# NIFTy-PPL/NIFTy

Hardware: AMD Instinct MI355X
Metric: MGVI iters/sec on 1024^3 RGSpace CorrelatedField, 8 samples; achieved HBM GB/s (higher is better)
Workload: dtype f32

## Files before the change

include/niftyk.h:

```cpp
#ifndef NIFTYK_H
#define NIFTYK_H
#include <stddef.h>
#include <stdint.h>

#ifdef __cplusplus
extern "C" {
#endif

typedef enum {
  NK_OK = 0,
  NK_ERR_INVALID = -1,
  NK_ERR_UNSUPPORTED = -2,
  NK_ERR_RUNTIME = -3,
  NK_ERR_NOMEM = -4
} nk_status;

typedef enum { NK_F32 = 0, NK_F64 = 1 } nk_dtype;

#define NK_HARTLEY_NON_CANONICAL 0
#define NK_HARTLEY_CANONICAL 1

enum { NK_PRO_PLAIN = 0, NK_PRO_AMP = 1, NK_PRO_AMP_JVP = 2, NK_PRO_MUL = 3 };
enum { NK_EPI_AFFINE = 0, NK_EPI_MUL = 1, NK_EPI_VJP = 2, NK_EPI_LIKELIHOOD = 3, NK_EPI_NONLIN = 4 };
enum { NK_LH_GAUSS = 0, NK_LH_POISSON = 1 };
enum { NK_NL_ID = 0, NK_NL_EXP = 1, NK_NL_SIGMOID = 2 };

typedef struct nk_fuse {
  int pro;
  const void* in;
  const void* in2;
  const int32_t* pidx;
  const double* amp;
  const double* damp;
  int epi;
  void* out;
  double scale;
  double offset;
  const void* mul;
  double mul_scalar;
  const void* xi;
  const void* addend;
  double addend_scale;
  int accumulate;
  double* abar;
  int lh_kind, nonlin;
  const void* data;
  const void* icov;
  double icov_scalar;
  void* out2;
  double* value;
  const void* afield;
  const void* dampT;
  int abar_copies;
  int64_t abar_stride;
  const void* dafield;
  double* w8;
  int field_octant;
  int value_slots;
  const int32_t* pidx_octant;
  const void* cg_r;
  const double* cg_scal;
  double* w8max;
  int pipe_chunks;
  void* const* pipe_wait;
  void* const* pipe_record;
  double* wfull;
  int io32;
  const void* carry1;
  const void* carry2;
} nk_fuse;

typedef struct nk_plan nk_plan;

const char* nk_last_error(void);
int nk_version(void);

int nk_plan_create(nk_plan** plan, int ndim, const int64_t* shape, int dtype, int64_t batch);
int nk_plan_destroy(nk_plan* plan);
size_t nk_plan_workspace_bytes(const nk_plan* plan);
int nk_hartley(const nk_plan* plan, const void* in, void* out, double scale, int convention, void* workspace,
               void* stream);
int nk_hartley_fused(const nk_plan* plan, const nk_fuse* fuse, int convention, void* workspace, void* stream);
int nk_plan_pipe_ok(const nk_plan* plan, int chunks);
int nk_plan_sandwich(const nk_plan* plan);
int nk_hartley_sandwich(const nk_plan* plan, const nk_fuse* fuse, double scale_first, int convention, void* workspace,
                        void* stream);
int nk_hartley_sandwich_pair(const nk_plan* plan, const nk_fuse* fuse_a, const nk_fuse* fuse_b, double scale_first,
                             int convention, void* workspace_a, void* workspace_b, void* stream);
int nk_fftn(const nk_plan* plan, const void* in, void* out, int inverse, double scale, void* workspace,
            void* stream);

int nk_profile_enable(int on);
int nk_profile_collect(double* ms, int64_t* count);

int nk_vdot(int64_t n, const void* a, const void* b, int dtype, double* result, int accumulate, void* stream);

int64_t nk_red_unit(int64_t n, int dtype);
int nk_red_layout(int64_t unit_elems, int k_local, int k_global, int seg_units, int seg_stride, int seg_off,
                  double* units_out);
int nk_red_finish(const double* units, int k_global, int nred, double* result, int accumulate, void* stream);
int nk_sum(int64_t n, const void* a, int dtype, double* result, int accumulate, void* stream);
int nk_stats(int64_t n, const void* a, int dtype, double* result3, void* stream);

enum { NK_OP_ADD = 0, NK_OP_SUB = 1, NK_OP_MUL = 2, NK_OP_DIV = 3 };
int nk_binary(int op, int64_t n, const void* a, double ascalar, const void* b, double bscalar, void* out,
              int dtype, void* stream);
int nk_cplx_muldiv(int64_t n, const void* a, int akind, double asr, double asi, const void* b, int bkind, double bsr,
                   double bsi, int conj_b, int divide, void* out, int dtype, void* stream);
int nk_cplx_pointwise(int fn, int64_t n, const void* x, void* out, int dtype, void* stream);
int nk_axpby(int64_t n, double alpha, const void* x, double beta, const void* y, void* out, int dtype,
             void* stream);
int nk_axpby_sqnorm(int64_t n, double alpha, const void* x, double beta, const void* y, void* out, int dtype, double* result,
                    int accumulate, void* stream);
int nk_pointwise(int fn, double param, int64_t n, const void* x, void* fx, void* dfx, int dtype, void* stream);
int nk_clip(double lo, double hi, int64_t n, const void* x, void* fx, void* dfx, int dtype, void* stream);
int nk_gather(int64_t n, const void* table, const int32_t* pidx, void* out, int dtype, void* stream);
int nk_scatter_add(int64_t n, const void* in, const int32_t* pidx, int64_t nbins, void* bins, int dtype,
                   void* stream);

int nk_csr_rowsum(int64_t nrows, const int64_t* rowptr, const int32_t* col, const float* wgt, const void* x, void* y,
                  int dtype, int lanes, void* stream);
int nk_spmv(int64_t nrows, const int64_t* rowptr, const int32_t* col, const float* wgt, const void* x, void* y, int dtype,
            void* stream);
int nk_spmv_t(int64_t nrows, const int64_t* rowptr, const int32_t* col, const float* wgt, const void* y, double* x64,
              int dtype, void* stream);

typedef struct nk_tiled_csr {
  int64_t n_rows, n_slots;
  int32_t n_items, ny, nx, th, tw;
  const int32_t* item_tile;
  const int64_t* item_blk;
  const int32_t* blk_slot;
  const int64_t* row_slot;
  const uint16_t* loc;
  const float* wgt;
} nk_tiled_csr;
int nk_tiled_rowsum(const nk_tiled_csr* m, int count, const void* const* x, void* const* y, double* scratch, int dtype,
                    void* stream);

int nk_roll(int ndim, const int64_t* shape, const int64_t* shift, int elem_bytes, const void* in, void* out, void* stream);

int nk_bluestein_rows(int64_t rows, int n, int m, const void* in, const void* w, const void* bhat_br, const void* tw, void* out,
                      double scale, int in_real, int out_hartley, int dtype, void* stream);

int nk_cumsum(int64_t n, const void* in, void* out, int reverse, int dtype, void* stream);

int nk_cplx_rows(int64_t rows, int64_t in_cols, int64_t out_cols, const void* a, const void* w, void* out, int mode,
                 double scale, int sgn, int dtype, void* stream);

int nk_fold_copies(int64_t n, int copies, int64_t stride, const double* src, double* dst, void* stream);

int nk_octant_expand(int ndim, const int64_t* shape, const void* table, const int32_t* pidx, void* field, int dtype,
                     int compact, void* stream);
int nk_octant_scatter(int ndim, const int64_t* shape, const double* w8, const int32_t* pidx, double* abar,
                      int merge_swapped_lines, void* stream);
int nk_octant_expand_k2(int ndim, const int64_t* shape, const double* table, const int32_t* bin_k2, int64_t nb, void* dense,
                        void* field8, int dtype, const int32_t* line_order, void* stream);
int nk_octant_scatter_k2(int ndim, const int64_t* shape, const double* w8, const int32_t* pidx, const int32_t* bin_k2,
                         int64_t nb, double* scratch, double* abar, const double* w8max, void* stream);
int nk_segment_sum(int64_t nseg, const int32_t* rowptr, const int32_t* perm, const double* src, double* dst, int accumulate,
                   void* stream);
int nk_plan_octant_vjp(const nk_plan* plan);

int nk_pindex_from_k2(int ndim, const int64_t* shape, const int32_t* k2table, int32_t* pidx, int64_t* rho,
                      void* stream);

int nk_cg_curv(int64_t n, const void* d, const void* q, int dtype, double* scal, int accumulate, void* stream);
int nk_cg_update(int64_t n, void* x, void* r, const void* d, const void* q, const void* b, int dtype,
                 double* scal, int accumulate, void* stream);
int nk_cg_update_dr(int64_t n, void* x, void* r, const void* d, const void* q, int dtype, double* scal, int accumulate,
                    void* stream);
int nk_cg_direction(int64_t n, void* d, const void* r, int dtype, double* scal, int roll, void* stream);

typedef struct nk_product {
  int nsub;
  int64_t size[3];
  const int32_t* pidx[3];
  const double* tab[3];
  const double* dtab[3];
  const double* scale;
  const double* dscale;
} nk_product;
int nk_product_field(const nk_product* p, int tangent, void* out, int dtype, void* stream);
int nk_mirror_combine(int ndim, const int64_t* shape, const int* group, int nsub, const double* coef, const void* in,
                      void* out, double scale, double offset, int dtype, void* stream);
size_t nk_product_marginal_scratch(const nk_product* p, int which);
int nk_product_marginal(const nk_product* p, int which, const double* w, double* scratch, double* marg, void* stream);

int nk_amp_forward(int nb, const double* geo, const double* hyp, const double* lat, double* state, double* amp,
                   void* stream);
int nk_amp_jvp(int nb, const double* geo, const double* hyp, const double* lat, double* state, const double* dlat,
               double* damp, void* stream);
int nk_amp_vjp(int nb, const double* geo, const double* hyp, const double* lat, double* state, const double* abar,
               double* latbar, void* stream);

int64_t nk_pcg64_normal_scratch_bytes(int64_t n, int attempt);
int nk_pcg64_normal(const uint64_t* state, const uint64_t* inc, int64_t n, double mean, double std, void* out, int dtype,
                    void* scratch, int64_t scratch_bytes, int attempt, uint64_t* status, void* stream);
int64_t nk_pcg64_fixed_scratch_bytes(void);
int nk_pcg64_uniform(const uint64_t* state, const uint64_t* inc, int64_t n, double low, double high, void* out, int dtype,
                     void* scratch, void* stream);
int nk_pcg64_pm1(const uint64_t* state, const uint64_t* inc, int64_t n, void* out, int dtype, int complex_units, void* scratch,
                 void* stream);

int64_t nk_pcg64_integers_scratch_bytes(int64_t nthreads);
int nk_pcg64_integers(const uint64_t* state, const uint64_t* inc, int64_t n, int64_t low, uint64_t rng, int64_t nthreads, int64_t* out,
                      void* scratch, uint64_t* status, void* stream);

#define NK_MAX_BATCH 8
int nk_plan_batch_ok(const nk_plan* plan);
int nk_hartley_fused_batch(const nk_plan* plan, const nk_fuse* fuse, int count, int convention, void* const* workspace,
                           void* stream);
int nk_amp_forward_batch(int nb, const double* geo, const double* hyp, int count, const double* const* lat,
                         double* const* state, double* const* amp, void* stream);
int nk_amp_jvp_batch(int nb, const double* geo, const double* hyp, int count, const double* const* lat, double* const* state,
                     const double* const* dlat, double* const* damp, void* stream);
int nk_amp_vjp_batch(int nb, const double* geo, const double* hyp, int count, const double* const* lat, double* const* state,
                     const double* const* abar, double* const* latbar, void* stream);
int nk_gather_batch(int64_t n, int count, const void* const* table, const int32_t* pidx, void* const* out, int dtype,
                    void* stream);
int nk_csr_rowsum_batch(int64_t nrows, const int64_t* rowptr, const int32_t* col, const float* wgt, int count,
                        const void* const* x, void* const* y, int dtype, int lanes, void* stream);
int nk_axpby_batch(int64_t n, int count, const double* alpha, const void* const* x, const double* beta,
                   const void* const* y, void* const* out, int dtype, void* stream);
int nk_axpby_sqnorm_batch(int64_t n, int count, const double* alpha, const void* const* x, const double* beta,
                          const void* const* y, void* const* out, int dtype, double* const* result, int accumulate,
                          void* stream);
int nk_binary_batch(int op, int64_t n, int count, const void* const* a, const double* ascalar, const void* const* b,
                    const double* bscalar, void* const* out, int dtype, void* stream);
int nk_vdot_batch(int64_t n, int count, const void* const* a, const void* const* b, int dtype, double* const* result,
                  int accumulate, void* stream);
int nk_sum_tree(int64_t n, int count, const void* const* term, void* out, int dtype, void* stream);
int nk_cg_curv_batch(int64_t n, int count, const void* const* d, const void* const* q, int dtype, double* const* scal,
                     int accumulate, void* stream);
int nk_cg_update_batch(int64_t n, int count, void* const* x, void* const* r, const void* const* d, const void* const* q,
                       const void* const* b, int dtype, double* const* scal, int accumulate, void* stream);
int nk_cg_update_dr_batch(int64_t n, int count, void* const* x, void* const* r, const void* const* d,
                          const void* const* q, int dtype, double* const* scal, int accumulate, void* stream);
int nk_cg_direction_batch(int64_t n, int count, void* const* d, const void* const* r, int dtype, double* const* scal,
                          int roll, void* stream);

// ... 25 lines not shown
```

nifty_amd/_lib.py:

```python
import ctypes
import os

_HERE = os.path.dirname(os.path.abspath(__file__))
LIB_PATH = os.environ.get("NK_LIB_PATH") or os.path.join(_HERE, "csrc", "libniftyk.so")

NK_OK, NK_ERR_INVALID, NK_ERR_UNSUPPORTED, NK_ERR_RUNTIME, NK_ERR_NOMEM = 0, -1, -2, -3, -4
NK_F32, NK_F64 = 0, 1
PRO_PLAIN, PRO_AMP, PRO_AMP_JVP, PRO_MUL = 0, 1, 2, 3
EPI_AFFINE, EPI_MUL, EPI_VJP, EPI_LIKELIHOOD, EPI_NONLIN = 0, 1, 2, 3, 4
LH_GAUSS, LH_POISSON = 0, 1
NL_ID, NL_EXP, NL_SIGMOID = 0, 1, 2
OP_ADD, OP_SUB, OP_MUL, OP_DIV = 0, 1, 2, 3

_vp, _i, _i64, _d, _sz = ctypes.c_void_p, ctypes.c_int, ctypes.c_int64, ctypes.c_double, ctypes.c_size_t


class Fuse(ctypes.Structure):

    _fields_ = [
        ("pro", _i), ("in_", _vp), ("in2", _vp), ("pidx", _vp), ("amp", _vp), ("damp", _vp),
        ("epi", _i), ("out", _vp), ("scale", _d), ("offset", _d), ("mul", _vp), ("mul_scalar", _d),
        ("xi", _vp), ("addend", _vp), ("addend_scale", _d), ("accumulate", _i), ("abar", _vp), ("lh_kind", _i), ("nonlin", _i), ("data", _vp),
        ("icov", _vp), ("icov_scalar", _d), ("out2", _vp), ("value", _vp),
        ("afield", _vp), ("dampT", _vp), ("abar_copies", _i), ("abar_stride", _i64), ("dafield", _vp), ("w8", _vp),
        ("field_octant", _i), ("value_slots", _i), ("pidx_octant", _vp), ("cg_r", _vp), ("cg_scal", _vp), ("w8max", _vp),
        ("pipe_chunks", _i), ("pipe_wait", _vp), ("pipe_record", _vp), ("wfull", _vp), ("io32", _i), ("carry1", _vp), ("carry2", _vp),
    ]


class Product(ctypes.Structure):

    _fields_ = [("nsub", _i), ("size", _i64 * 3), ("pidx", _vp * 3), ("tab", _vp * 3), ("dtab", _vp * 3), ("scale", _vp),
                ("dscale", _vp)]


class TiledCsr(ctypes.Structure):

    _fields_ = [("n_rows", _i64), ("n_slots", _i64), ("n_items", ctypes.c_int32), ("ny", ctypes.c_int32), ("nx", ctypes.c_int32),
                ("th", ctypes.c_int32), ("tw", ctypes.c_int32), ("item_tile", _vp), ("item_blk", _vp), ("blk_slot", _vp),
                ("row_slot", _vp), ("loc", _vp), ("wgt", _vp)]


class NufftPlan(ctypes.Structure):

    _i32 = ctypes.c_int32
    _fields_ = [("ndim", _i32), ("w", _i32), ("beta", _d), ("n", _i32 * 3), ("nmodes", _i32 * 3), ("tile", _i32 * 3),
                ("ntiles", _i32 * 3), ("reach", _i32 * 3), ("m", _i64), ("u", _vp), ("perm", _vp), ("bin_start", _vp),
                ("n_items", _i64), ("item", _vp), ("n_split", _i64), ("split_tile", _vp), ("split_slab", _vp), ("corr", _vp)]


SIGNATURES = {
    "nk_last_error": (ctypes.c_char_p, []),
    "nk_version": (_i, []),
    "nk_plan_create": (_i, [ctypes.POINTER(_vp), _i, ctypes.POINTER(_i64), _i, _i64]),
    "nk_plan_destroy": (_i, [_vp]),
    "nk_plan_workspace_bytes": (_sz, [_vp]),
    "nk_hartley": (_i, [_vp, _vp, _vp, _d, _i, _vp, _vp]),
    "nk_hartley_fused": (_i, [_vp, ctypes.POINTER(Fuse), _i, _vp, _vp]),
    "nk_plan_sandwich": (_i, [_vp]),
    "nk_plan_pipe_ok": (_i, [_vp, _i]),
    "nk_hartley_sandwich": (_i, [_vp, ctypes.POINTER(Fuse), _d, _i, _vp, _vp]),
    "nk_hartley_sandwich_pair": (_i, [_vp, ctypes.POINTER(Fuse), ctypes.POINTER(Fuse), _d, _i, _vp, _vp, _vp]),
    "nk_fftn": (_i, [_vp, _vp, _vp, _i, _d, _vp, _vp]),
    "nk_profile_enable": (_i, [_i]),
    "nk_profile_collect": (_i, [_vp, _vp]),
    "nk_vdot": (_i, [_i64, _vp, _vp, _i, _vp, _i, _vp]),
    "nk_product_field": (_i, [ctypes.POINTER(Product), _i, _vp, _i, _vp]),
    "nk_mirror_combine": (_i, [_i, ctypes.POINTER(_i64), ctypes.POINTER(_i), _i, ctypes.POINTER(_d), _vp, _vp, _d, _d, _i, _vp]),
    "nk_product_marginal_scratch": (_sz, [ctypes.POINTER(Product), _i]),
    "nk_product_marginal": (_i, [ctypes.POINTER(Product), _i, _vp, _vp, _vp, _vp]),
    "nk_red_unit": (_i64, [_i64, _i]),
    "nk_red_layout": (_i, [_i64, _i, _i, _i, _i, _i, _vp]),
    "nk_red_finish": (_i, [_vp, _i, _i, _vp, _i, _vp]),
    "nk_sum": (_i, [_i64, _vp, _i, _vp, _i, _vp]),
    "nk_stats": (_i, [_i64, _vp, _i, _vp, _vp]),
    "nk_binary": (_i, [_i, _i64, _vp, _d, _vp, _d, _vp, _i, _vp]),
    "nk_cplx_muldiv": (_i, [_i64, _vp, _i, _d, _d, _vp, _i, _d, _d, _i, _i, _vp, _i, _vp]),
    "nk_cplx_pointwise": (_i, [_i, _i64, _vp, _vp, _i, _vp]),
    "nk_axpby": (_i, [_i64, _d, _vp, _d, _vp, _vp, _i, _vp]),
    "nk_axpby_sqnorm": (_i, [_i64, _d, _vp, _d, _vp, _vp, _i, _vp, _i, _vp]),
    "nk_pointwise": (_i, [_i, _d, _i64, _vp, _vp, _vp, _i, _vp]),
    "nk_clip": (_i, [_d, _d, _i64, _vp, _vp, _vp, _i, _vp]),
    "nk_gather": (_i, [_i64, _vp, _vp, _vp, _i, _vp]),
    "nk_scatter_add": (_i, [_i64, _vp, _vp, _i64, _vp, _i, _vp]),
    "nk_octant_expand": (_i, [_i, ctypes.POINTER(_i64), _vp, _vp, _vp, _i, _i, _vp]),
    "nk_octant_scatter": (_i, [_i, ctypes.POINTER(_i64), _vp, _vp, _vp, _i, _vp]),
    "nk_octant_expand_k2": (_i, [_i, ctypes.POINTER(_i64), _vp, _vp, _i64, _vp, _vp, _i, _vp, _vp]),
    "nk_segment_sum": (_i, [_i64, _vp, _vp, _vp, _vp, _i, _vp]),
    "nk_octant_scatter_k2": (_i, [_i, ctypes.POINTER(_i64), _vp, _vp, _vp, _i64, _vp, _vp, _vp, _vp]),
    "nk_plan_octant_vjp": (_i, [_vp]),
    "nk_fold_copies": (_i, [_i64, _i, _i64, _vp, _vp, _vp]),
    "nk_cumsum": (_i, [_i64, _vp, _vp, _i, _i, _vp]),
    "nk_cplx_rows": (_i, [_i64, _i64, _i64, _vp, _vp, _vp, _i, _d, _i, _i, _vp]),
    "nk_csr_rowsum": (_i, [_i64, _vp, _vp, _vp, _vp, _vp, _i, _i, _vp]),
    "nk_tiled_rowsum": (_i, [ctypes.POINTER(TiledCsr), _i, _vp, _vp, _vp, _i, _vp]),
    "nk_bluestein_rows": (_i, [_i64, _i, _i, _vp, _vp, _vp, _vp, _vp, _d, _i, _i, _i, _vp]),
    "nk_roll": (_i, [_i, ctypes.POINTER(_i64), ctypes.POINTER(_i64), _i, _vp, _vp, _vp]),
    "nk_spmv": (_i, [_i64, _vp, _vp, _vp, _vp, _vp, _i, _vp]),
    "nk_spmv_t": (_i, [_i64, _vp, _vp, _vp, _vp, _vp, _i, _vp]),
    "nk_pindex_from_k2": (_i, [_i, ctypes.POINTER(_i64), _vp, _vp, _vp, _vp]),
    "nk_cg_curv": (_i, [_i64, _vp, _vp, _i, _vp, _i, _vp]),
    "nk_cg_update": (_i, [_i64, _vp, _vp, _vp, _vp, _vp, _i, _vp, _i, _vp]),
    "nk_cg_update_dr": (_i, [_i64, _vp, _vp, _vp, _vp, _i, _vp, _i, _vp]),
    "nk_pcg64_normal_scratch_bytes": (_i64, [_i64, _i]),
    "nk_pcg64_normal": (_i, [_vp, _vp, _i64, _d, _d, _vp, _i, _vp, _i64, _i, _vp, _vp]),
    "nk_pcg64_fixed_scratch_bytes": (_i64, []),
    "nk_pcg64_uniform": (_i, [_vp, _vp, _i64, _d, _d, _vp, _i, _vp, _vp]),
    "nk_pcg64_pm1": (_i, [_vp, _vp, _i64, _vp, _i, _i, _vp, _vp]),
    "nk_pcg64_integers_scratch_bytes": (_i64, [_i64]),
    "nk_pcg64_integers": (_i, [_vp, _vp, _i64, _i64, ctypes.c_uint64, _i64, _vp, _vp, _vp, _vp]),
    "nk_cg_direction": (_i, [_i64, _vp, _vp, _i, _vp, _i, _vp]),
    "nk_amp_forward": (_i, [_i, _vp, _vp, _vp, _vp, _vp, _vp]),
    "nk_amp_jvp": (_i, [_i, _vp, _vp, _vp, _vp, _vp, _vp, _vp]),
    "nk_amp_vjp": (_i, [_i, _vp, _vp, _vp, _vp, _vp, _vp, _vp]),
    "nk_nufft_spread": (_i, [ctypes.POINTER(NufftPlan), _vp, _vp, _vp, _i, _vp]),
    "nk_nufft_interp": (_i, [ctypes.POINTER(NufftPlan), _vp, _vp, _i, _vp]),
    "nk_nufft_crop": (_i, [ctypes.POINTER(NufftPlan), _vp, _vp, _i, _vp]),
    "nk_nufft_pad": (_i, [ctypes.POINTER(NufftPlan), _vp, _i, _vp, _i, _vp]),
    "nk_plan_batch_ok": (_i, [_vp]),
    "nk_hartley_fused_batch": (_i, [_vp, ctypes.POINTER(Fuse), _i, _i, _vp, _vp]),
    "nk_amp_forward_batch": (_i, [_i, _vp, _vp, _i, _vp, _vp, _vp, _vp]),
    "nk_amp_jvp_batch": (_i, [_i, _vp, _vp, _i, _vp, _vp, _vp, _vp, _vp]),
    "nk_amp_vjp_batch": (_i, [_i, _vp, _vp, _i, _vp, _vp, _vp, _vp, _vp]),
    "nk_gather_batch": (_i, [_i64, _i, _vp, _vp, _vp, _i, _vp]),
    "nk_csr_rowsum_batch": (_i, [_i64, _vp, _vp, _vp, _i, _vp, _vp, _i, _i, _vp]),
    "nk_axpby_batch": (_i, [_i64, _i, _vp, _vp, _vp, _vp, _vp, _i, _vp]),
    "nk_axpby_sqnorm_batch": (_i, [_i64, _i, _vp, _vp, _vp, _vp, _vp, _i, _vp, _i, _vp]),
    "nk_binary_batch": (_i, [_i, _i64, _i, _vp, _vp, _vp, _vp, _vp, _i, _vp]),
    "nk_vdot_batch": (_i, [_i64, _i, _vp, _vp, _i, _vp, _i, _vp]),
    "nk_sum_tree": (_i, [_i64, _i, _vp, _vp, _i, _vp]),
    "nk_cg_curv_batch": (_i, [_i64, _i, _vp, _vp, _i, _vp, _i, _vp]),
    "nk_cg_update_batch": (_i, [_i64, _i, _vp, _vp, _vp, _vp, _vp, _i, _vp, _i, _vp]),
    "nk_cg_update_dr_batch": (_i, [_i64, _i, _vp, _vp, _vp, _vp, _i, _vp, _i, _vp]),
    "nk_cg_direction_batch": (_i, [_i64, _i, _vp, _vp, _i, _vp, _i, _vp]),
}
MAX_BATCH = 8


def ptr_array(tensors):
    return (_vp * len(tensors))(*[None if t is None else t.data_ptr() for t in tensors])


def double_array(values):
    return (_d * len(values))(*[float(v) for v in values])

_lib = None


class NiftykError(RuntimeError):
    pass


def load():
    global _lib
    if _lib is not None:
        return _lib
    if not os.path.exists(LIB_PATH):
        raise NiftykError(
            f"{LIB_PATH} not found: the HIP extension is not built. Run `python -c 'import __graft_entry__ as g; "
            "g.build()'` (hipcc --offload-arch=gfx950). nifty_amd has no CPU fallback for device fields."
        )
    lib = ctypes.CDLL(LIB_PATH)
    for name, (res, args) in SIGNATURES.items():
        fn = getattr(lib, name)
        fn.restype = res
        fn.argtypes = args
    _lib = lib
    return lib


def check(rc, what=""):
    if rc == NK_OK:
        return
    msg = load().nk_last_error().decode(errors="replace")
    text = f"{what}: {msg}" if what else msg
    if rc == NK_ERR_INVALID:
        raise ValueError(text)
    if rc == NK_ERR_UNSUPPORTED:
        raise NotImplementedError(text)
    if rc == NK_ERR_NOMEM:
        raise MemoryError(text)
    raise NiftykError(text)
```

nifty_amd/backend.py:

```python
import ctypes
import math
import os

import numpy as np
import torch

from . import _lib as L
from . import config

_DT = {torch.float32: L.NK_F32, torch.float64: L.NK_F64}
_plans = {}


_raw_stream = getattr(torch._C, "_cuda_getCurrentRawStream", None)


_current_device = torch.cuda.current_device


def _stream():
    if _raw_stream is not None:
        return _raw_stream(_current_device())
    return torch.cuda.current_stream().cuda_stream

# ... 82 lines not shown
    except NotImplementedError:
        _unsupported.add(key)
        return False
    return True


_chirps = {}
_CHIRP_MAX = 1 << 14


def _chirp(n, cdt, inverse, device):
    key = (n, cdt, bool(inverse), device.index)
    ent = _chirps.get(key)
    if ent is None:
        m = 1 << (2 * n - 2).bit_length()
        if m > _CHIRP_MAX:
            raise NotImplementedError(f"axis of length {n} is too long for the chirp-z fallback")
        k = torch.arange(n, dtype=torch.int64)
        ang = (k * k % (2 * n)).to(torch.float64) * (math.pi / n)
        w = torch.polar(torch.ones(n, dtype=torch.float64), ang if inverse else -ang)
        b = torch.zeros(m, dtype=torch.complex128)
        b[:n] = w.conj()
        b[m - n + 1:] = w.conj()[1:].flip(0)
        w, b = w.to(cdt).to(device), b.to(cdt).to(device)
        rdt = torch.float32 if cdt == torch.complex64 else torch.float64
        get_plan((m,), rdt, 1, device)
        ent = _chirps[key] = (m, w, fftn(b, ndim=1))
    return ent


BLUESTEIN_LDS_BYTES = 64 * 1024
_blu_tables = {}


def _bluestein_tables(n, m, cdt, inverse, device):
    key = (n, m, cdt, bool(inverse), device.index)
    ent = _blu_tables.get(key)
    if ent is None:
        k = np.arange(n, dtype=np.int64)
        ang = (k * k % (2 * n)).astype(np.float64) * (np.pi / n)
        w = np.exp(1j * ang if inverse else -1j * ang)
        b = np.zeros(m, dtype=np.complex128)
        b[:n] = w.conj()
        b[m - n + 1:] = w.conj()[1:][::-1]
        bhat = np.fft.fft(b)
        bits = m.bit_length() - 1
        rev = np.zeros(m, dtype=np.int64)
        for bit in range(bits):
            rev |= ((np.arange(m) >> bit) & 1) << (bits - 1 - bit)
        tw = np.exp(-2j * np.pi * np.arange(m // 2) / m)
        npdt = np.complex64 if cdt == torch.complex64 else np.complex128
        ent = _blu_tables[key] = tuple(torch.from_numpy(np.ascontiguousarray(a.astype(npdt))).to(device) for a in (w, bhat[rev], tw))
    return ent


def cplx_rows(a, w, in_cols, out_cols, mode, scale=1.0, sgn=1):
    _require_device(a, w)
    rows = a.numel() // max(1, in_cols)
    if mode == 2:
        rdt = torch.float32 if a.dtype == torch.complex64 else torch.float64
        out = torch.empty(a.shape[:-1] + (out_cols,), dtype=rdt, device=a.device)
    else:
        cdt = a.dtype if a.is_complex() else (torch.complex64 if a.dtype == torch.float32 else torch.complex128)
        out = torch.empty(a.shape[:-1] + (out_cols,), dtype=cdt, device=a.device)
    code = 0 if out.dtype in (torch.float32, torch.complex64) else 1
    L.check(L.load().nk_cplx_rows(rows, in_cols, out_cols, a.data_ptr(), ptr(w), out.data_ptr(), mode, float(scale),
                                  int(sgn), code, _stream()), "nk_cplx_rows")
    return out


def _fft_last_axis_any(z, inverse, real_in=False, hartley=0, scale=1.0):
    n = z.shape[-1]
    rdt = z.dtype if real_in else (torch.float32 if z.dtype == torch.complex64 else torch.float64)
    cdt = torch.complex64 if rdt == torch.float32 else torch.complex128
    batch = z.numel() // max(1, n)
    m = 1 << max(2, (2 * n - 2).bit_length())
    native = n == 1 or z.numel() == 0 or plan_supported((n,), rdt, batch, z.device)
    if (not native and m * (8 if rdt == torch.float32 else 16) <= BLUESTEIN_LDS_BYTES and os.environ.get("NK_BLUESTEIN", "1") != "0"):
        w, bhat_br, tw = _bluestein_tables(n, m, cdt, inverse, z.device)
        out = torch.empty(z.shape, dtype=rdt if hartley else cdt, device=z.device)
        L.check(L.load().nk_bluestein_rows(batch, n, m, z.data_ptr(), w.data_ptr(), bhat_br.data_ptr(), tw.data_ptr(), out.data_ptr(),
                                           float(scale) if hartley else 1.0, 1 if real_in else 0, int(hartley),
                                           0 if rdt == torch.float32 else 1, _stream()), "nk_bluestein_rows")
        return out
    if real_in:
        z = cplx_rows(z, None, n, n, 1)
    if n == 1 or z.numel() == 0:
        res = z.clone()
    elif native:
        res = fftn(z, ndim=1, inverse=inverse)
    else:
        if m > _CHIRP_MAX or not plan_supported((m,), rdt, batch, z.device) or not plan_supported((m,), rdt, 1, z.device):
            raise NotImplementedError(f"axis of length {n} is too long for the chirp-z fallback")
        m, w, fb = _chirp(n, z.dtype, inverse, z.device)
        a = cplx_rows(z, w, n, m, 0)
        p = cplx_rows(fftn(a, ndim=1), fb, m, m, 0)
        c = fftn(p, ndim=1, inverse=True, scale=1.0 / m)
        res = cplx_rows(c, w, m, n, 0)
    return cplx_rows(res, None, n, n, 2, scale, hartley) if hartley else res


def _fft_any(z, ndim, inverse, real_in=False, hartley=0, scale=1.0):
    first, last = z.dim() - ndim, z.dim() - 1
    for ax in range(first, z.dim()):
        z = _fft_last_axis_any(z.movedim(ax, -1).contiguous(), inverse, real_in=real_in and ax == first,
                               hartley=hartley if ax == last else 0, scale=scale).movedim(-1, ax)
    return z.contiguous()


def _convention():
    return 0 if config.get("hartley_convention") == "non_canonical_hartley" else 1


def hartley(x, ndim=None, scale=1.0, out=None):
    _require_device(x)
    x = x.contiguous()
    ndim = x.dim() if ndim is None else ndim
    shape = x.shape[x.dim() - ndim:]
    batch = x.numel() // max(1, int(torch.Size(shape).numel()))
    if not plan_supported(shape, x.dtype, batch, x.device):
        h = _fft_any(x, ndim, False, real_in=True, hartley=1 if _convention() == 0 else -1, scale=scale)
        return h if out is None else out.copy_(h)
    plan = get_plan(shape, x.dtype, batch, x.device)
    out = torch.empty_like(x) if out is None else out
    L.check(L.load().nk_hartley(plan.handle, x.data_ptr(), out.data_ptr(), float(scale), _convention(),
                                plan.workspace.data_ptr(), _stream()), "nk_hartley")
    return out


def hartley_fused(plan, fuse):
    if plan.device.index != _current_device():
        _wrong_device(plan.device.index)
    L.check(L.load().nk_hartley_fused(plan.handle, ctypes.byref(fuse), _convention(), plan.workspace.data_ptr(),
                                      _stream()), "nk_hartley_fused")


def plan_sandwich(plan):
    return bool(L.load().nk_plan_sandwich(plan.handle))


def hartley_sandwich(plan, fuse, scale_first):
    if plan.device.index != _current_device():
        _wrong_device(plan.device.index)
    L.check(L.load().nk_hartley_sandwich(plan.handle, ctypes.byref(fuse), float(scale_first), _convention(),
                                         plan.workspace.data_ptr(), _stream()), "nk_hartley_sandwich")


def hartley_sandwich_pair(plan, fuse_a, fuse_b, scale_first, workspace_b):
    if plan.device.index != _current_device():
        _wrong_device(plan.device.index)
    L.check(L.load().nk_hartley_sandwich_pair(plan.handle, ctypes.byref(fuse_a), ctypes.byref(fuse_b), float(scale_first),
                                              _convention(), plan.workspace.data_ptr(), workspace_b.data_ptr(), _stream()),
            "nk_hartley_sandwich_pair")


def fftn(x, ndim=None, inverse=False, scale=1.0):
    _require_device(x)
    if not x.is_complex():
        raise TypeError("fftn expects a complex tensor")
    x = x.contiguous()
    ndim = x.dim() if ndim is None else ndim
    shape = x.shape[x.dim() - ndim:]
    batch = x.numel() // max(1, int(torch.Size(shape).numel()))
    rdt = torch.float32 if x.dtype == torch.complex64 else torch.float64
    if not plan_supported(shape, rdt, batch, x.device):
        f = _fft_any(x, ndim, inverse)
        return f if float(scale) == 1.0 else cplx_rows(f, None, f.shape[-1], f.shape[-1], 0, scale)
    plan = get_plan(shape, rdt, batch, x.device)
    out = torch.empty_like(x)
    L.check(L.load().nk_fftn(plan.handle, torch.view_as_real(x).data_ptr(), torch.view_as_real(out).data_ptr(),
                             1 if inverse else 0, float(scale), plan.workspace.data_ptr(), _stream()), "nk_fftn")
    return out


def new_scalar(device, n=1):
    return torch.zeros(n, dtype=torch.float64, device=device)


def vdot(a, b, result=None, accumulate=False):
    _require_device(a, b)
    if a.numel() != b.numel() or a.dtype != b.dtype:
        raise ValueError("vdot: shape/dtype mismatch")
    result = new_scalar(a.device) if result is None else result
    L.check(L.load().nk_vdot(a.numel(), a.data_ptr(), b.data_ptr(), dtype_code(a), result.data_ptr(),
                             1 if accumulate else 0, _stream()), "nk_vdot")
    return result


def vsum(a, result=None, accumulate=False):
    _require_device(a)
    result = new_scalar(a.device) if result is None else result
    L.check(L.load().nk_sum(a.numel(), a.data_ptr(), dtype_code(a), result.data_ptr(), 1 if accumulate else 0,
                            _stream()), "nk_sum")
    return result


def binary(op, a, b, out=None):
    ta, tb = torch.is_tensor(a), torch.is_tensor(b)
    ref = a if ta else b
    _require_device(ref)
    if ta and tb and (a.shape != b.shape or a.dtype != b.dtype):
        raise ValueError("binary: shape/dtype mismatch")
    out = torch.empty_like(ref) if out is None else out
    L.check(L.load().nk_binary(op, ref.numel(), ptr(a) if ta else 0, 0.0 if ta else float(a), ptr(b) if tb else 0,
                               0.0 if tb else float(b), out.data_ptr(), dtype_code(ref), _stream()), "nk_binary")
    return out


def _cplx_operand(x, cdt):
    if torch.is_tensor(x):
        if x.is_complex():
            return x.to(cdt).contiguous(), 0, 0.0, 0.0
        rdt = torch.float32 if cdt == torch.complex64 else torch.float64
        return x.to(rdt).contiguous(), 1, 0.0, 0.0
    z = complex(x)
    return None, 2, z.real, z.imag


def cplx_muldiv(a, b, divide=False, conj_b=False):
    tensors = [t for t in (a, b) if torch.is_tensor(t)]
    _require_device(*tensors)
    wide = any(t.dtype in (torch.complex128, torch.float64) for t in tensors)
    cdt = torch.complex128 if wide else torch.complex64
    ta, ka, ar, ai = _cplx_operand(a, cdt)
    tb, kb, br, bi = _cplx_operand(b, cdt)
    shape = tensors[0].shape
    if any(t.shape != shape for t in tensors):
        raise ValueError("cplx_muldiv: shape mismatch")
    out = torch.empty(shape, dtype=cdt, device=tensors[0].device)
    L.check(L.load().nk_cplx_muldiv(out.numel(), ptr(ta), ka, ar, ai, ptr(tb), kb, br, bi, int(bool(conj_b)), int(bool(divide)),
                                    out.data_ptr(), 0 if cdt == torch.complex64 else 1, _stream()), "nk_cplx_muldiv")
    return out


CPLX_POINTWISE = {"exp": 0, "log": 1, "sqrt": 2, "reciprocal": 3, "conjugate": 4, "abs": 5, "absolute": 5}


def cplx_pointwise(op, x):
    _require_device(x)
    x = x.contiguous()
    fn = CPLX_POINTWISE[op]
    rdt = torch.float32 if x.dtype == torch.complex64 else torch.float64
    out = torch.empty(x.shape, dtype=rdt if fn == 5 else x.dtype, device=x.device)
    L.check(L.load().nk_cplx_pointwise(fn, x.numel(), x.data_ptr(), out.data_ptr(), 0 if x.dtype == torch.complex64 else 1,
                                       _stream()), "nk_cplx_pointwise")
    return out


def axpby(alpha, x, beta=0.0, y=None, out=None):
    _require_device(x, y)
    out = torch.empty_like(x) if out is None else out
    L.check(L.load().nk_axpby(x.numel(), float(alpha), x.data_ptr(), float(beta), ptr(y), out.data_ptr(), dtype_code(x),
                              _stream()), "nk_axpby")
    return out


def axpby_sqnorm(alpha, x, beta, y, result, accumulate=False):
    _require_device(x, y, result)
    out = torch.empty_like(x)
    L.check(L.load().nk_axpby_sqnorm(x.numel(), float(alpha), x.data_ptr(), float(beta), y.data_ptr(), out.data_ptr(),
                                     dtype_code(x), result.data_ptr(), 1 if accumulate else 0, _stream()), "nk_axpby_sqnorm")
    return out


POINTWISE = {"exp": 0, "log": 1, "sqrt": 2, "tanh": 3, "sigmoid": 4, "reciprocal": 5, "power": 6, "abs": 7,
             "absolute": 7, "log1p": 8, "expm1": 9, "arctan": 10, "sin": 11, "cos": 12, "tan": 13, "sinc": 14, "log10": 15,
             "sinh": 16, "cosh": 17, "sign": 18, "softplus": 19, "exponentiate": 20, "unitstep": 21, "clip": 22}


def pointwise(name, x, param=0.0, want_derivative=False, param2=None):
    _require_device(x)
    fx = torch.empty_like(x)
    dfx = torch.empty_like(x) if want_derivative else None
    if name == "clip":
        lo = -math.inf if param is None else float(param)
        hi = math.inf if param2 is None else float(param2)
        L.check(L.load().nk_clip(lo, hi, x.numel(), x.data_ptr(), fx.data_ptr(), ptr(dfx), dtype_code(x), _stream()), "nk_clip")
    else:
        L.check(L.load().nk_pointwise(POINTWISE[name], float(param), x.numel(), x.data_ptr(), fx.data_ptr(), ptr(dfx),
                                      dtype_code(x), _stream()), "nk_pointwise")
    return (fx, dfx) if want_derivative else fx


def gather(table, pidx, out_shape, out=None):
    _require_device(table, pidx)
    out = torch.empty(out_shape, dtype=table.dtype, device=table.device) if out is None else out
    L.check(L.load().nk_gather(out.numel(), table.data_ptr(), pidx.data_ptr(), out.data_ptr(), dtype_code(table),
                               _stream()), "nk_gather")
    return out


def scatter_add(x, pidx, nbins):
    _require_device(x, pidx)
    bins = torch.zeros(nbins, dtype=torch.float64, device=x.device)
    L.check(L.load().nk_scatter_add(x.numel(), x.data_ptr(), pidx.data_ptr(), nbins, bins.data_ptr(), dtype_code(x),
                                    _stream()), "nk_scatter_add")
    return bins


def lanes_for(nnz, nrows):
    avg = nnz / max(1, nrows)
    return 1 if avg <= 4 else 4 if avg <= 32 else 16 if avg <= 256 else 64


BIN_PLAN_MAX = 1 << 28

# ... 217 lines not shown
    lib = L.load()
    status = torch.empty(2, dtype=torch.int64, device=device)

    def draw(state, inc, need, lo, span, nthreads):
        words = (ctypes.c_uint64 * 4)(state >> 64, state & (2**64 - 1), inc >> 64, inc & (2**64 - 1))
        scratch = torch.empty(lib.nk_pcg64_integers_scratch_bytes(nthreads), dtype=torch.uint8, device=device)
        dst = out[n - need:]
        L.check(lib.nk_pcg64_integers(ctypes.addressof(words), ctypes.addressof(words) + 16, need, lo, span, nthreads, dst.data_ptr(),
                                      scratch.data_ptr(), status.data_ptr(), _stream()), "nk_pcg64_integers")
        used, err = status.cpu().tolist()
        return dst, int(used), bool(err & 2)

    first, _ = _bounded_integers(rng, low, high, n, draw)
    if n and int(high) == int(low):
        out.fill_(int(low))
    elif first:
        out[:len(first)] = torch.tensor(first, dtype=torch.int64)
    return out.reshape(tuple(shape))


def pcg64_normal(rng, mean, std, shape, dtype, device):
    import ctypes

    import numpy as np

    bg = rng.bit_generator
    st = bg.state
    if st.get("bit_generator") != "PCG64":
        raise TypeError("pcg64_normal needs a numpy Generator over PCG64 (np.random.default_rng)")
    if float(std) < 0:
        raise ValueError("scale < 0")
    n = int(np.prod(shape, dtype=np.int64)) if len(tuple(shape)) else 1
    out = torch.empty(tuple(shape), dtype=dtype, device=device)
    _require_device(out)
    if n == 0:
        return out
    state, inc = int(st["state"]["state"]), int(st["state"]["inc"])
    words = (ctypes.c_uint64 * 4)(state >> 64, state & (2**64 - 1), inc >> 64, inc & (2**64 - 1))
    status = torch.empty(2, dtype=torch.int64, device=device)
    lib = L.load()
    for attempt in range(9):
        nbytes = lib.nk_pcg64_normal_scratch_bytes(n, attempt)
        scratch = torch.empty(nbytes, dtype=torch.uint8, device=device)
        L.check(lib.nk_pcg64_normal(ctypes.addressof(words), ctypes.addressof(words) + 16, n, float(mean), float(std),
                                    out.data_ptr(), dtype_code(out), scratch.data_ptr(), nbytes, attempt,
                                    status.data_ptr(), _stream()), "nk_pcg64_normal")
        consumed, err = status.cpu().tolist()
        del scratch
        if err == 0:
            break
        if err & 1:
            raise RuntimeError("nk_pcg64_normal: chain merge failed")
    else:
        raise RuntimeError("nk_pcg64_normal: scratch sizing failed")
    st["state"]["state"] = _pcg64_advanced(state, inc, int(consumed))
    bg.state = st
    return out


def _pcg64_words(rng):
    bg = rng.bit_generator
    st = bg.state
    if st.get("bit_generator") != "PCG64":
        raise TypeError("needs a numpy Generator over PCG64 (np.random.default_rng)")
    import ctypes

    state, inc = int(st["state"]["state"]), int(st["state"]["inc"])
    words = (ctypes.c_uint64 * 4)(state >> 64, state & (2**64 - 1), inc >> 64, inc & (2**64 - 1))
    return bg, st, state, inc, words


def pcg64_uniform(rng, low, high, shape, dtype, device):
    import ctypes

    import numpy as np

    bg, st, state, inc, words = _pcg64_words(rng)
    n = int(np.prod(shape, dtype=np.int64)) if len(tuple(shape)) else 1
    out = torch.empty(tuple(shape), dtype=dtype, device=device)
    _require_device(out)
    if n == 0:
        return out
    lib = L.load()
    scratch = torch.empty(lib.nk_pcg64_fixed_scratch_bytes(), dtype=torch.uint8, device=device)
    L.check(lib.nk_pcg64_uniform(ctypes.addressof(words), ctypes.addressof(words) + 16, n, float(low), float(high),
                                 out.data_ptr(), dtype_code(out), scratch.data_ptr(), _stream()), "nk_pcg64_uniform")
    st["state"]["state"] = _pcg64_advanced(state, inc, n)
    bg.state = st
    return out


def pcg64_pm1(rng, shape, dtype, device, complex_units=False):
    import ctypes

    import numpy as np

    n = int(np.prod(shape, dtype=np.int64)) if len(tuple(shape)) else 1
    cdt = {torch.float32: torch.complex64, torch.float64: torch.complex128}[dtype]
    out = torch.empty(tuple(shape), dtype=cdt if complex_units else dtype, device=device)
    _require_device(out)
    if n == 0:
        return out
    flat = (torch.view_as_real(out) if complex_units else out).reshape(-1)
    width = 2 if complex_units else 1
    done = 0
    if rng.bit_generator.state["has_uint32"]:
        v = int(rng.integers(0, 4 if complex_units else 2))
        first = ([1, 0], [0, 1], [-1, 0], [0, -1])[v] if complex_units else [2 * v - 1]
        flat[:width] = torch.tensor(first, dtype=dtype, device=device)
        done = 1
    m = n - done
    if m > 0:
        bg, st, state, inc, words = _pcg64_words(rng)
        lib = L.load()
        scratch = torch.empty(lib.nk_pcg64_fixed_scratch_bytes(), dtype=torch.uint8, device=device)
        L.check(lib.nk_pcg64_pm1(ctypes.addressof(words), ctypes.addressof(words) + 16, m, flat[done * width:].data_ptr(),
                                 _DT[dtype], 1 if complex_units else 0, scratch.data_ptr(), _stream()), "nk_pcg64_pm1")
        nraw = (m + 1) // 2
        if m % 2:
            st["state"]["state"] = _pcg64_advanced(state, inc, nraw - 1)
            bg.state = st
            last = int(bg.random_raw(1)[0])
            st = bg.state
            st["has_uint32"], st["uinteger"] = 1, last >> 32
            bg.state = st
        else:
            st["state"]["state"] = _pcg64_advanced(state, inc, nraw)
            st["has_uint32"], st["uinteger"] = 0, 0
            bg.state = st
    return out


def _runs_on_operand_device(fn):
    import functools

    @functools.wraps(fn)
    def wrapper(*args, **kw):
        for a in args:
            if torch.is_tensor(a):
                if a.is_cuda and a.device.index != _current_device():
                    with torch.cuda.device(a.device):
                        return fn(*args, **kw)
                break
            if isinstance(a, (Plan, PlanView)):
                if a.device.index != _current_device():
                    with torch.cuda.device(a.device):
                        return fn(*args, **kw)
                break
        return fn(*args, **kw)

    return wrapper


for _name in ("cplx_rows", "cplx_pointwise", "hartley", "hartley_fused", "hartley_sandwich", "hartley_sandwich_pair", "fftn", "vdot", "vsum", "binary", "axpby",
              "axpby_sqnorm",
              "pointwise", "gather", "scatter_add", "bin_plan", "bin_sum", "spmv", "spmv_t", "stats", "cumsum"):
    globals()[_name] = _runs_on_operand_device(globals()[_name])
del _name
```

nifty_amd/csrc/nk_fft.hip:

```cpp
#include <hip/hip_runtime.h>

#include <algorithm>

#include <cstdio>
#include <cstring>
#include <new>

#include "nk_fft_batch.h"

#include <mutex>
#include <vector>
using ProfScope = NkProfScope;
thread_local const NkBatchCtx* t_batch = nullptr;

template <typename T>
__device__ __forceinline__ void nk_run_stages(C2<T>* lds, int tid, int nthr, const NkLinePlan& lp, const NkTile& tl,
                                              const C2<T>* __restrict__ tw) {
  int L = lp.n;
  for (int s = 0; s < lp.nstage; ++s) {
    const int R = lp.radix[s];
    NK_STAGE_DISPATCH(R, lds, tid, nthr, lp, tl, L, tw, s)
    L /= R;
    __syncthreads();
  }
// ... 125 lines not shown
  NkFuse fs = f;
  pf.blk0 = 0;
  if (pf.a_cnt > 0) {
    if (pf.g.batch != 1 || (xmap_env & 4)) return nk_set_error(NK_ERR_UNSUPPORTED, "staged final pass: batch 1, natural block order");
    pf.blk0 = (int64_t)pf.a0 * pf.tiles_per_a;
    blocks = (int64_t)pf.a_cnt * pf.tiles_per_a;
    const int64_t off = pf.blk0 * ((CT::THREADS + 63) / 64);
    if (fs.value_slots > 0) {
      if (fs.value) fs.value += off;
      if (fs.w8max) fs.w8max += off;
      fs.value_slots = fs.value_slots > off ? (int)(fs.value_slots - off) : 0;
      if (fs.value_slots == 0) return nk_set_error(NK_ERR_RUNTIME, "final pass: more wavefronts than reduction slots (nk_value_slot_count)");
    }
  }
  if (fs.value_slots > 0 && blocks * ((CT::THREADS + 63) / 64) > fs.value_slots)
    return nk_set_error(NK_ERR_RUNTIME, "final pass: more wavefronts than reduction slots (nk_value_slot_count)");
  if (t_batch != nullptr) {
    if constexpr (nk_twin_final<NL, COUPLES, EC, PAIR>()) {
      if (pf.a_cnt > 0 || pf.g.batch != 1) return nk_set_error(NK_ERR_UNSUPPORTED, "batched final pass: one unstaged grid per member");
      return nk_twin_launch_final<T, NL, COUPLES, EC>(pf, blocks, tw, xmap_env & 4, st);
    } else {
      return nk_set_error(NK_ERR_UNSUPPORTED, "batched final pass: no batched twin of this kernel class");
    }
  }
  return nk_launch<k2_final<T, NL, COUPLES, EC, PAIR>>("k2_final", dim3((unsigned)blocks), dim3(CT::THREADS), CT::LDS_BYTES, st, pf, fs, tw,
                                                       work, xmap_env & 4);
}

template <typename T, int NL>
static int nk_launch_final(const NkPassF& pf, const NkFuse& f, const C2<T>* tw, const C2<T>* work, hipStream_t st) {
  if (nk_knobs().ec_generic && !f.field_octant) {
    if (f.epi == NK_EPI_VJP) return nk_launch_final_c<T, NL, true, -1>(pf, f, tw, work, st);
    return nk_launch_final_c<T, NL, false, -1>(pf, f, tw, work, st);
  }
  if (f.epi == NK_EPI_VJP && f.afield) {
    if constexpr (nk_final_single_2d<T, NL>())
      if (pf.A == 1) return nk_launch_final_c<T, NL, false, 2>(pf, f, tw, work, st);
    return nk_launch_final_c<T, NL, true, 2>(pf, f, tw, work, st);
  }
  if (f.epi == NK_EPI_VJP) return nk_launch_final_c<T, NL, true, -1>(pf, f, tw, work, st);
  if (f.epi == NK_EPI_AFFINE) return nk_launch_final_c<T, NL, false, 0>(pf, f, tw, work, st);
  if (f.epi == NK_EPI_MUL) return nk_launch_final_c<T, NL, false, 1>(pf, f, tw, work, st);
  if (f.epi == NK_EPI_LIKELIHOOD) {
    if constexpr (sizeof(T) == 8)
      if (f.io32) return nk_launch_final_c<T, NL, false, 5>(pf, f, tw, work, st);
    return nk_launch_final_c<T, NL, false, 3>(pf, f, tw, work, st);
  }
  return nk_launch_final_c<T, NL, false, -1>(pf, f, tw, work, st);
}

template <typename T, int NL>
static int nk_launch_final3(const NkPassF& pf, const NkFuse& f, const C2<T>* tw, const C2<T>* work, hipStream_t st) {
  if (f.epi == NK_EPI_VJP && f.afield) return nk_launch_final_c<T, NL, true, 2, 1>(pf, f, tw, work, st);
  if (f.epi == NK_EPI_VJP) return nk_launch_final_c<T, NL, true, -1, 1>(pf, f, tw, work, st);
  if (f.epi == NK_EPI_AFFINE) return nk_launch_final_c<T, NL, false, 0, 1>(pf, f, tw, work, st);
  return nk_launch_final_c<T, NL, false, -1, 1>(pf, f, tw, work, st);
}

template <typename T>
static int nk_dispatch_final3(int nl, const NkPassF& pf, const NkFuse& f, const C2<T>* tw, const C2<T>* work,
                              hipStream_t st) {
  return nk_dispatch_fast(nl, "no fast final pass for this length", [&](auto N) { return nk_launch_final3<T, N()>(pf, f, tw, work, st); });
}

template <typename T>
static int nk_dispatch_final_pair(int nl, const NkPassF& pf, const NkFuse& fa, const NkFuse& fb, const C2<T>* tw,
                                  const C2<T>* worka, const C2<T>* workb, hipStream_t st) {
  return nk_dispatch_fast(nl, "no fast final pass for this length",
                          [&](auto N) { return nk_launch_final_pair<T, N()>(pf, fa, fb, tw, worka, workb, st); });
}

template <typename T>
static int nk_dispatch_final(int nl, const NkPassF& pf, const NkFuse& f, const C2<T>* tw, const C2<T>* work,
                             hipStream_t st) {
  return nk_dispatch_fast(nl, "no fast final pass for this length", [&](auto N) { return nk_launch_final<T, N()>(pf, f, tw, work, st); });
}

template <typename T, int H, bool IS_1D>
static int nk_launch_contig(const NkPassA& pa, const NkFuse& f, const C2<T>* tw, const C2<T>* twr, C2<T>* work,
                            hipStream_t st) {
  using CT = ContigTile<T, H>;
  const int64_t blocks = (pa.nlines + CT::TILE - 1) / CT::TILE;
  return nk_launch<k2_contig<T, H, IS_1D>>("k2_contig", dim3((unsigned)blocks), dim3(CT::THREADS), CT::LDS_BYTES, st, pa, f, tw, twr, work);
}

template <typename T, int N, int MODE, int PC>
static int nk_launch_strided_pc(NkPassS ps, const NkFuse& f, const C2<T>* tw, C2<T>* work, C2<T>* scratch, hipStream_t st) {
  using ST = StridedTile<T, N, nk_strided_cx<MODE, PC>(), MODE>;
  ps.tl.tile = ST::TILE;
  ps.tl.dtile = nk_make_div(ST::TILE);
  ps.tiles_per_slab = (int)(ps.inner / ST::TILE);
  const int64_t blocks = ps.outer * ps.tiles_per_slab;
  const int xmap_env = nk_knobs().xmap;
  const int xmap = MODE == 3 ? (xmap_env & 1) : ((xmap_env & 2) | ((xmap_env & 8) && ps.blo > 0 ? 2 : 0));
  if (t_batch != nullptr) {
    if constexpr (MODE != 3 || !nk_twin_strided<N, PC>()) {
      return nk_set_error(NK_ERR_UNSUPPORTED, "batched strided pass: no batched twin of this kernel class");
    } else {
      return nk_twin_launch_strided<T, N, PC>(ps, blocks, tw, xmap, st);
    }
  }
  return nk_launch<k2_strided<T, N, MODE, PC>>("k2_strided", dim3((unsigned)blocks), dim3(ST::THREADS), ST::LDS_TOTAL, st, ps, f, tw, work,
                                               scratch, xmap);
}

template <typename T, bool IS_1D>
static int nk_dispatch_contig(int h, const NkPassA& pa, const NkFuse& f, const C2<T>* tw, const C2<T>* twr, C2<T>* work,
                              hipStream_t st) {
  return nk_dispatch_fast(h, "no fast contiguous pass for this length",
                          [&](auto N) { return nk_launch_contig<T, N(), IS_1D>(pa, f, tw, twr, work, st); });
}

template <typename T, int N, int MODE>
static int nk_launch_strided(const NkPassS& ps, const NkFuse& f, const C2<T>* tw, C2<T>* work, C2<T>* scratch, hipStream_t st) {
  if constexpr (MODE == 3) {
    if constexpr (sizeof(T) == 8)
      if (f.field_octant && f.pro == NK_PRO_AMP && f.io32) return nk_launch_strided_pc<T, N, MODE, 9>(ps, f, tw, work, scratch, st);
    if (f.field_octant && f.pro == NK_PRO_AMP) return nk_launch_strided_pc<T, N, MODE, 4>(ps, f, tw, work, scratch, st);
    if (f.field_octant && f.pro == NK_PRO_AMP_JVP) return nk_launch_strided_pc<T, N, MODE, 5>(ps, f, tw, work, scratch, st);
    if (f.pro == NK_PRO_PLAIN) return nk_launch_strided_pc<T, N, MODE, 0>(ps, f, tw, work, scratch, st);
    if (f.pro == NK_PRO_MUL) return nk_launch_strided_pc<T, N, MODE, 6>(ps, f, tw, work, scratch, st);
    if (f.pro == NK_PRO_AMP && f.afield) return nk_launch_strided_pc<T, N, MODE, 1>(ps, f, tw, work, scratch, st);
    if (f.pro == NK_PRO_AMP_JVP && f.afield && f.dafield)
      return nk_launch_strided_pc<T, N, MODE, 3>(ps, f, tw, work, scratch, st);
    if (f.pro == NK_PRO_AMP_JVP && f.afield && f.dampT)
      return nk_launch_strided_pc<T, N, MODE, 2>(ps, f, tw, work, scratch, st);
  }
  return nk_launch_strided_pc<T, N, MODE, -1>(ps, f, tw, work, scratch, st);
}

template <typename T, int MODE>
static int nk_dispatch_strided(int n, const NkPassS& ps, const NkFuse& f, const C2<T>* tw, C2<T>* work, C2<T>* scratch,
                               hipStream_t st) {
  return nk_dispatch_fast(n, "no fast strided pass for this length",
                          [&](auto N) { return nk_launch_strided<T, N(), MODE>(ps, f, tw, work, scratch, st); });
}

#ifndef NK_CONTIG3_WAVES
#define NK_CONTIG3_WAVES 0
#endif
#if NK_CONTIG3_WAVES > 0
#define NK_CONTIG3_ATTR __attribute__((amdgpu_waves_per_eu(1, NK_CONTIG3_WAVES)))
#else
#define NK_CONTIG3_ATTR
#endif
template <typename T, int H, int PC>
__global__ void __launch_bounds__((Contig3Tile<T, H>::THREADS)) NK_CONTIG3_ATTR
    k3_contig(NkPass3 p, NkFuse f, const C2<T>* __restrict__ tw, const C2<T>* __restrict__ twr, C2<T>* __restrict__ work) {
  extern __shared__ __align__(16) unsigned char smem[];
  DeviceExec<T, Contig3Tile<T, H>::SC::E> ex;
  nk_contig3_body<T, H, Contig3Tile<T, H>::TILE, PC>(ex, p, f, blockIdx.x, (T*)smem, tw, twr, work);
}

#ifndef NK_QUAD_MAXW_F64_5
#define NK_QUAD_MAXW_F64_5 4
#endif
#ifndef NK_QUAD_MAXW_F64_8
#define NK_QUAD_MAXW_F64_8 8
#endif
#ifndef NK_QUAD_MAXW_F32_5
#define NK_QUAD_MAXW_F32_5 8
#endif
#ifndef NK_QUAD_MAXW_F32_8
#define NK_QUAD_MAXW_F32_8 8
#endif
template <typename T, int PC>
constexpr int nk_quad_max_waves() {
  return sizeof(T) == 8 ? (PC == 8 ? NK_QUAD_MAXW_F64_8 : NK_QUAD_MAXW_F64_5) : (PC == 8 ? NK_QUAD_MAXW_F32_8 : NK_QUAD_MAXW_F32_5);
}
template <typename T, int H, int PC>
__global__ void __launch_bounds__((Contig3Tile<T, H>::QTHREADS))
    k3_contig_quad(NkPass3 p, NkFuse f, const C2<T>* __restrict__ tw, const C2<T>* __restrict__ twr, C2<T>* __restrict__ work) {
  extern __shared__ __align__(16) unsigned char smem[];
  DeviceExec<T, Contig3Tile<T, H>::SC::E> ex;
  nk_contig3_body<T, H, 4, PC, true>(ex, p, f, (int64_t)blockIdx.x + p.blk0, (T*)smem, tw, twr, work, (int)blockIdx.y);
}
template <typename T, int H, int PC, int MAXW>
__global__ void __launch_bounds__((Contig3Tile<T, H>::QTHREADS)) __attribute__((amdgpu_waves_per_eu(1, MAXW)))
    k3_contig_quad_w(NkPass3 p, NkFuse f, const C2<T>* __restrict__ tw, const C2<T>* __restrict__ twr, C2<T>* __restrict__ work) {
  extern __shared__ __align__(16) unsigned char smem[];
  DeviceExec<T, Contig3Tile<T, H>::SC::E> ex;
  nk_contig3_body<T, H, 4, PC, true>(ex, p, f, (int64_t)blockIdx.x + p.blk0, (T*)smem, tw, twr, work, (int)blockIdx.y);
}
template <typename T, int H, int PC>
static constexpr auto nk_quad_kernel() {
  if constexpr (nk_quad_max_waves<T, PC>() < 8)
    return k3_contig_quad_w<T, H, PC, nk_quad_max_waves<T, PC>()>;
  else
    return k3_contig_quad<T, H, PC>;
}

template <typename T, int H, int PC>
static int nk_launch_contig3(const NkPass3& p3, const NkFuse& f, const C2<T>* tw, const C2<T>* twr, C2<T>* work, hipStream_t st) {
  using CT = Contig3Tile<T, H>;
  if constexpr ((PC == 4 || PC == 5 || PC == 7 || PC == 8) && CT::QUAD_OK) {
    if (nk_contig3_quad(p3.nblk, p3.g.ndim)) {
      const int64_t batch = p3.nlines / ((int64_t)p3.g.na * p3.g.nm);
      int64_t qblocks = batch * (p3.g.na / 2 + 1) * (p3.g.nm / 2 + 1);
      if (p3.nblk > 0) {
        if (batch != 1 || p3.blk0 < 0 || p3.blk0 + p3.nblk > qblocks) return nk_set_error(NK_ERR_INVALID, "k3_contig_quad: bad stage range");
        qblocks = p3.nblk;
      }
      const int64_t per = (int64_t)(p3.g.na / 2 + 1) * (p3.g.nm / 2 + 1);
      const int64_t gx = p3.nblk > 0 ? qblocks : per;
      if (gx > 0x7fffffffLL || batch > 65535) return nk_set_error(NK_ERR_UNSUPPORTED, "too many lines for one launch");
      NkPass3 pq = p3;
      pq.dmh = nk_make_div(p3.g.nm / 2 + 1);
      return nk_launch<nk_quad_kernel<T, H, PC>()>("k3_contig_quad", dim3((unsigned)gx, (unsigned)(p3.nblk > 0 ? 1 : batch)), dim3(CT::QTHREADS),
                                                   CT::QLDS_BYTES, st, pq, f, tw, twr, work);
    }
  }
  if (p3.nblk > 0)
    return nk_set_error(NK_ERR_UNSUPPORTED, "nk_fuse.pipe_chunks: the staged first pass exists for the QUAD launches only (3-D plan, "
                                             "octant prologue classes, last axis <= 2048 fp32, NK_CONTIG_QUAD != 0)");
  const int64_t blocks = (p3.nlines + CT::TILE - 1) / CT::TILE;
  if (blocks > 0x7fffffffLL) return nk_set_error(NK_ERR_UNSUPPORTED, "too many lines for one launch");
  return nk_launch<k3_contig<T, H, PC>>("k3_contig", dim3((unsigned)blocks), dim3(CT::THREADS), CT::LDS_BYTES, st, p3, f, tw, twr, work);
}

template <typename T, int H>
static int nk_launch_contig3_pc(const NkPass3& p3, const NkFuse& f, const C2<T>* tw, const C2<T>* twr, C2<T>* work, hipStream_t st) {
  if (f.field_octant && f.pro == NK_PRO_AMP) return nk_launch_contig3<T, H, 4>(p3, f, tw, twr, work, st);
  if (f.field_octant && f.pro == NK_PRO_AMP_JVP && f.cg_r && f.dafield) return nk_launch_contig3<T, H, 8>(p3, f, tw, twr, work, st);
  if (f.field_octant && f.pro == NK_PRO_AMP_JVP && f.pidx_octant && f.dampT) return nk_launch_contig3<T, H, 7>(p3, f, tw, twr, work, st);
  if (f.field_octant && f.pro == NK_PRO_AMP_JVP) return nk_launch_contig3<T, H, 5>(p3, f, tw, twr, work, st);
  if (f.pro == NK_PRO_PLAIN) return nk_launch_contig3<T, H, 0>(p3, f, tw, twr, work, st);
  if (f.pro == NK_PRO_MUL) return nk_launch_contig3<T, H, 6>(p3, f, tw, twr, work, st);
  return nk_launch_contig3<T, H, -1>(p3, f, tw, twr, work, st);
}

template <typename T>
static int nk_dispatch_contig3(int h, const NkPass3& p3, const NkFuse& f, const C2<T>* tw, const C2<T>* twr, C2<T>* work,
                               hipStream_t st) {
  return nk_dispatch_fast(h, "no fast contiguous pass for this length",
                          [&](auto N) { return nk_launch_contig3_pc<T, N()>(p3, f, tw, twr, work, st); });
}

#ifndef NK_MID_CX
#define NK_MID_CX 1
#endif
#ifndef NK_MID_WAVES
#define NK_MID_WAVES 0
#endif
#ifndef NK_MID_PF
#define NK_MID_PF 0
#endif
#ifndef NK_MID_WIDE_XM
#define NK_MID_WIDE_XM 2
#endif
#ifndef NK_MID_WIDE
#define NK_MID_WIDE 0
#endif
#ifndef NK_MID_TWO
#define NK_MID_TWO 1
#endif
#ifndef NK_MID_TWO_MF
#define NK_MID_TWO_MF 0
#endif
template <typename T, int N, bool MF>
struct MidCfg {
  static constexpr bool WIDE = NK_MID_WIDE && SchedW<T, N>::E == 64;
  static constexpr bool TWO = NK_MID_TWO && !WIDE && (!MF || NK_MID_TWO_MF) && sizeof(T) == 4 && Sched<T, N>::E == 32 &&
                              StridedTile<T, N, false, 3>::THREADS == 512 && StridedTile<T, N, false, 3>::LDS_BYTES <= 64 * 1024;
  using ST = StridedTile<T, N, !WIDE && !TWO && NK_MID_CX != 0, WIDE ? 0 : 3>;
  using SC = typename ST::SC;
  static constexpr int XM = WIDE ? NK_MID_WIDE_XM : (ST::CPLX ? 1 : 0);
  static constexpr bool TWC = TWO;
  static constexpr int WAVES = NK_MID_WAVES > 0 ? NK_MID_WAVES : TWO ? 4 : ST::THREADS <= 256 ? 2 : 1;
};
template <typename T, int N, bool MF>
__global__ void __launch_bounds__((MidCfg<T, N, MF>::ST::THREADS), (MidCfg<T, N, MF>::WAVES))
    k3_mid(NkPassM pm, NkFuse f, const C2<T>* __restrict__ tw, C2<T>* __restrict__ work, int64_t nblk, int xmap) {
  extern __shared__ __align__(16) unsigned char smem[];
  using CF = MidCfg<T, N, MF>;
  using ST = typename CF::ST;
  DeviceExecR<MidRegs<T, CF::SC::E, NK_MID_PF != 0>> ex;
  C2<T>* tw_lds = ST::TWLDS ? reinterpret_cast<C2<T>*>(smem + ST::LDS_BYTES) : nullptr;
  nk_mid_body<T, N, ST::TILE, CF::XM, MF, NK_MID_PF != 0, typename CF::SC, CF::TWC>(ex, pm, f, (int64_t)blockIdx.x, (int64_t)gridDim.x,
                                                                                     nblk, xmap, (T*)smem, tw, work, tw_lds);
}

template <typename T, int N, bool MF>
static int nk_launch_mid(NkPassM pm, const NkFuse& f, const C2<T>* tw, C2<T>* work, hipStream_t st) {
  using ST = typename MidCfg<T, N, MF>::ST;
  pm.s.tl.tile = ST::TILE;
  pm.s.tl.dtile = nk_make_div(ST::TILE);
  pm.s.tiles_per_slab = (int)(pm.s.inner / ST::TILE);
  const int64_t blocks = pm.s.outer * pm.s.tiles_per_slab;
  int64_t grid = blocks;
  if (NK_MID_PF) {
    static int cus = 0;
    if (cus == 0) {
      int dev = 0;
      hipDeviceProp_t prop;
      cus = (hipGetDevice(&dev) == hipSuccess && hipGetDeviceProperties(&prop, dev) == hipSuccess) ? prop.multiProcessorCount : 256;
    }
    const int per_cu_env = nk_knobs().mid_wg_per_cu;
    const int per_cu = per_cu_env > 0 ? per_cu_env : (ST::LDS_TOTAL <= 80 * 1024 && ST::THREADS <= 512 ? 2 : 1);
    if (grid > (int64_t)cus * per_cu) grid = (int64_t)cus * per_cu;
  }
  return nk_launch<k3_mid<T, N, MF>>("k3_mid", dim3((unsigned)grid), dim3(ST::THREADS), ST::LDS_TOTAL, st, pm, f, tw, work, blocks,
                                     nk_knobs().xmap & 2);
}

template <typename T>
static int nk_dispatch_mid(int n, const NkPassM& pm, const NkFuse& f, const C2<T>* tw, C2<T>* work, hipStream_t st) {
  return nk_dispatch_fast(n, "no fast strided pass for this length", [&](auto N) {
    return f.mul ? nk_launch_mid<T, N(), true>(pm, f, tw, work, st) : nk_launch_mid<T, N(), false>(pm, f, tw, work, st);
  });
}

struct NkPassCC {
  NkLinePlan lp;
  NkTile tl;
  int64_t nlines;
  int swap;
  double scale;
  NkDiv dn;
};

template <typename T>
__global__ void __launch_bounds__(nk_gen_max_threads<T>()) k_c2c_contig(NkPassCC p, const C2<T>* __restrict__ tw, const C2<T>* __restrict__ in,
// ... 543 lines not shown
  __shared__ double red[4];
  const double* slots = sa.slots[blockIdx.y];
  if (!slots) return;
  double* part = sa.slots[blockIdx.y] + n;
  const int64_t per = (n + gridDim.x - 1) / gridDim.x;
  const int64_t lo = (int64_t)blockIdx.x * per, hi = lo + per < n ? lo + per : n;
  double v = 0.0;
  for (int64_t i = lo + threadIdx.x; i < hi; i += 256) v += slots[i];
  const double s = nk_fold_block_sum(v, red);
  if (threadIdx.x == 0) part[blockIdx.x] = s;
}
__global__ void __launch_bounds__(NK_FOLD_BLOCKS) k_fold_slots_b_b(NkSlotArr sa, int64_t n) {
  __shared__ double red[NK_FOLD_BLOCKS / 64];
  if (!sa.slots[blockIdx.y]) return;
  const double* part = sa.slots[blockIdx.y] + n;
  const double s = nk_fold_block_sum(part[threadIdx.x], red);
  if (threadIdx.x == 0) *sa.value[blockIdx.y] += s;
}

static bool nk_same_class(const nk_fuse& a, const nk_fuse& b) {
  return a.pro == b.pro && a.epi == b.epi && !a.afield == !b.afield && !a.dafield == !b.dafield && !a.dampT == !b.dampT &&
         a.field_octant == b.field_octant && !a.io32 == !b.io32 && !a.w8 == !b.w8 && !a.wfull == !b.wfull &&
         a.abar_copies == b.abar_copies && !a.pidx_octant == !b.pidx_octant;
}

extern "C" int nk_plan_batch_ok(const nk_plan* P) {
  if (!P || !nk_plan_uses_pipeline2(P)) return 0;
  const NkHostPlan& hp = P->hp;
  if (hp.g.ndim != 2 || hp.g.batch != 1) return 0;
  return P->hp.dtype == NK_F32 ? nk_fast_strided_ok<float>(hp.g.na, hp.pc.inner) : nk_fast_strided_ok<double>(hp.g.na, hp.pc.inner);
}

template <typename T>
static int nk_run_hartley_batch(const nk_plan* P, const nk_fuse* fuse, int count, int convention, void* const* workspace,
                                hipStream_t st) {
  const NkHostPlan& hp = P->hp;
  NkBatchCtx bc;
  bc.count = count;
  bc.fuse = fuse;
  for (int m = 0; m < NK_MAX_BATCH; ++m) {
    const int k = m < count ? m : 0;
    bc.wa.work[m] = workspace[k];
    bc.wa.scratch[m] = (char*)workspace[k] + (hp.work_bytes + 255) / 256 * 256;
  }
  NkPipe2 q = nk_pipe2_setup(hp, convention == NK_HARTLEY_CANONICAL ? -1 : 1, nk_knobs().work_blo, nk_knobs().work_pad);
  {
    const int64_t smax = q.s1.ss > q.s0.inner ? q.s1.ss : q.s0.inner;
    if (128 * (smax > q.s1.inner ? smax : q.s1.inner) * (int64_t)sizeof(C2<T>) >= ((int64_t)1 << 32))
      return nk_set_error(NK_ERR_UNSUPPORTED, "transform too large for the 32-bit thread offsets of the strided passes");
  }
  const int64_t n = nk_value_slot_count(hp);
  NkSlotArr sa;
  bool any = false;
  for (int m = 0; m < NK_MAX_BATCH; ++m) {
    sa.slots[m] = nullptr, sa.value[m] = nullptr;
    if (m >= count) {
      bc.final_fuse[m] = fuse[0];
      continue;
    }
    NkFuse f2 = fuse[m];
    if (f2.w8max && f2.w8 && f2.epi == NK_EPI_VJP)
      return nk_set_error(NK_ERR_UNSUPPORTED, "nk_fuse.w8max: only the 3-D final pass reports max |w8|");
    f2.w8max = nullptr;
    if (f2.value && (f2.epi == NK_EPI_LIKELIHOOD || f2.epi == NK_EPI_VJP)) {
      sa.slots[m] = nk_value_slots(hp, workspace[m]);
      sa.value[m] = f2.value;
      f2.value = sa.slots[m];
      f2.value_slots = (int)std::min<int64_t>(n, 0x7fffffff);
      any = true;
    }
    bc.final_fuse[m] = f2;
  }
  struct Scope {
    Scope(const NkBatchCtx* b) { t_batch = b; }
    ~Scope() { t_batch = nullptr; }
  } scope(&bc);
  int rc;
  {
    NkProfScope ps(st, 1, fuse[0].pro, fuse[0].epi, count);
    int n1, n2;
    if (nk_tl_split<T>(hp.g, n1, n2))
      rc = nk_tl_first_axis<T>(q.s1, n1, n2, fuse[0], (const C2<T>*)P->d_tw_t64, (const C2<T>*)(n2 == 64 ? P->d_tw_t64 : P->d_tw_t32),
                               (const C2<T>*)P->d_tw_c, (C2<T>*)bc.wa.work[0], st);
    else
      rc = nk_dispatch_strided<T, 3>(hp.g.na, q.s1, fuse[0], (const C2<T>*)P->d_tw_c, (C2<T>*)bc.wa.work[0], (C2<T>*)bc.wa.scratch[0], st);
  }
  if (rc != NK_OK) return rc;
  if (any) {
    hipLaunchKernelGGL(k_zero_slots_b, dim3(64, count), dim3(256), 0, st, sa, n);
    rc = nk_check_launch("k_zero_slots_b");
    if (rc != NK_OK) return rc;
  }
  {
    NkProfScope ps(st, 3, fuse[0].pro, fuse[0].epi, count);
    rc = nk_dispatch_final<T>(hp.g.nl, q.pf, bc.final_fuse[0], (const C2<T>*)P->d_tw_f, (const C2<T>*)bc.wa.work[0], st);
  }
  if (rc != NK_OK || !any) return rc;
  hipLaunchKernelGGL(k_fold_slots_a_b, dim3(NK_FOLD_BLOCKS, count), dim3(256), 0, st, sa, n);
  hipLaunchKernelGGL(k_fold_slots_b_b, dim3(1, count), dim3(NK_FOLD_BLOCKS), 0, st, sa, n);
  return nk_check_launch("k_fold_slots_b");
}

extern "C" int nk_hartley_fused_batch(const nk_plan* P, const nk_fuse* fuse, int count, int convention, void* const* workspace,
                                      void* stream) {
  if (!P || !fuse || !workspace || count < 1 || count > NK_MAX_BATCH)
    return nk_set_error(NK_ERR_INVALID, "nk_hartley_fused_batch: bad argument (1 <= count <= NK_MAX_BATCH)");
  for (int m = 0; m < count; ++m) {
    const int rc = nk_fused_check(P, fuse + m, convention);
    if (rc != NK_OK) return rc;
    if (!workspace[m]) return nk_set_error(NK_ERR_INVALID, "nk_hartley_fused_batch: every member needs a workspace");
    for (int k = 0; k < m; ++k)
      if (workspace[k] == workspace[m]) return nk_set_error(NK_ERR_INVALID, "nk_hartley_fused_batch: members share a workspace");
    if (!nk_same_class(fuse[0], fuse[m]))
      return nk_set_error(NK_ERR_INVALID, "nk_hartley_fused_batch: the members select different kernel classes");
  }
  hipStream_t st = (hipStream_t)stream;
  if (count == 1 || !nk_plan_batch_ok(P) || !nk_batch_class_ok(P->hp.g, fuse[0])) {
    for (int m = 0; m < count; ++m) {
      const int rc = P->hp.dtype == NK_F32 ? nk_run_hartley<float>(P, fuse[m], convention, workspace[m], st)
                                           : nk_run_hartley<double>(P, fuse[m], convention, workspace[m], st);
      if (rc != NK_OK) return rc;
    }
    return NK_OK;
  }
  if (P->hp.dtype == NK_F32) return nk_run_hartley_batch<float>(P, fuse, count, convention, workspace, st);
  return nk_run_hartley_batch<double>(P, fuse, count, convention, workspace, st);
}

static bool nk_strided_tile_divides(const nk_plan* P, int n, int64_t inner) {
  return P->hp.dtype == NK_F32 ? nk_fast_strided_ok<float>(n, inner) : nk_fast_strided_ok<double>(n, inner);
}
extern "C" int nk_plan_sandwich(const nk_plan* P) {
  if (!P || !nk_plan_uses_pipeline2(P) || !nk_fast_contig_ok(P->hp.g.h)) return 0;
  const NkGeom& g = P->hp.g;
  const int64_t rs = g.h + (P->hp.dtype == NK_F32 ? nk_pipe3_colpad<float>() : nk_pipe3_colpad<double>());
  if (g.ndim == 3 && !nk_strided_tile_divides(P, g.nm, rs)) return 0;
  return nk_strided_tile_divides(P, g.na, g.ndim == 3 ? (int64_t)g.nm * rs : rs) ? 1 : 0;
}

template <typename T>
static bool nk_contig3_quad_ok(int h) {
  return nk_with_fast_size(h, false, [](auto N) { return (bool)Contig3Tile<T, N()>::QUAD_OK; });
}
extern "C" int nk_plan_pipe_ok(const nk_plan* P, int chunks) {
  if (!nk_plan_sandwich(P) || chunks < 2 || (chunks & 1)) return 0;
  const NkGeom& g = P->hp.g;
  if (g.ndim != 3 || g.batch != 1 || g.na % chunks != 0) return 0;
  if (!nk_knobs().contig_quad || (nk_knobs().xmap & 4)) return 0;
  return (P->hp.dtype == NK_F32 ? nk_contig3_quad_ok<float>(g.h) : nk_contig3_quad_ok<double>(g.h)) ? 1 : 0;
}

template <typename T>
static int nk_run_sandwich(const nk_plan* P, const NkFuse& f, double scale_first, int convention, void* workspace, hipStream_t st,
                           bool with_final = true, NkPipe3* q_out = nullptr) {
  const NkHostPlan& hp = P->hp;
  const int sign = convention == NK_HARTLEY_CANONICAL ? -1 : 1;
  const int work_pad = nk_knobs().work_pad;
  const NkPipe3 q = nk_pipe3_setup<T>(hp, sign, work_pad, scale_first * (f.mul_scalar != 0.0 ? f.mul_scalar : 1.0));
  if (q_out) *q_out = q;
  if (nk_pipe3_work_elems(hp.g, nk_pipe3_colpad<T>(), work_pad) * sizeof(C2<T>) > hp.work_bytes)
    return nk_set_error(NK_ERR_RUNTIME, "nk_hartley_sandwich: plan workspace too small");
  if (128 * (q.ss > q.pm.s.inner ? q.ss : q.pm.s.inner) * (int64_t)sizeof(C2<T>) >= ((int64_t)1 << 32))
    return nk_set_error(NK_ERR_UNSUPPORTED, "transform too large for the 32-bit thread offsets of the strided passes");
  C2<T>* work = (C2<T>*)workspace;
  int rc;
  const int C = f.pipe_chunks >= 2 ? f.pipe_chunks : 0;
  if (C) {
    if (hp.g.ndim != 3 || hp.g.batch != 1 || (C & 1) || hp.g.na % C != 0 || !f.field_octant ||
        (f.pro != NK_PRO_AMP && f.pro != NK_PRO_AMP_JVP))
      return nk_set_error(NK_ERR_UNSUPPORTED, "nk_fuse.pipe_chunks: needs a 3-D plan with batch 1, an even chunk count that divides "
                                               "the first axis, and an octant amplitude prologue");
  }
  const int wc = C ? hp.g.na / C : 0;
  if (C) {
    const int Mh = hp.g.nm / 2 + 1;
    for (int j = 0; j < C / 2; ++j) {
      if (f.pipe_wait) {
        hipError_t e = hipStreamWaitEvent(st, (hipEvent_t)f.pipe_wait[j], 0);
        if (e != hipSuccess) return nk_set_hip_error(e, "hipStreamWaitEvent(pipe_wait)");
      }
      NkPass3 p1 = q.p1;
      const int a_lo = j * wc, a_hi = (j == C / 2 - 1) ? hp.g.na / 2 + 1 : (j + 1) * wc;
      p1.blk0 = (int64_t)a_lo * Mh;
      p1.nblk = (int64_t)(a_hi - a_lo) * Mh;
      ProfScope ps(st, 5, f.cg_r ? 4 : f.pro, f.epi);
      rc = nk_dispatch_contig3<T>(hp.g.h, p1, f, (const C2<T>*)P->d_tw_a, (const C2<T>*)P->d_twr_a, work, st);
      if (rc != NK_OK) return rc;
    }
  } else {
    ProfScope ps(st, 5, f.cg_r ? 4 : f.pro, f.epi);
    rc = nk_dispatch_contig3<T>(hp.g.h, q.p1, f, (const C2<T>*)P->d_tw_a, (const C2<T>*)P->d_twr_a, work, st);
    if (rc != NK_OK) return rc;
  }
  if (hp.g.ndim == 3) {
    ProfScope ps(st, 6, f.pro, f.epi);
    rc = nk_dispatch_strided<T, 0>(hp.g.nm, q.s2, f, (const C2<T>*)P->d_tw_b, work, (C2<T>*)nullptr, st);
    if (rc != NK_OK) return rc;
  }
  {
    ProfScope ps(st, 7, f.pro, f.epi);
    rc = nk_dispatch_mid<T>(hp.g.na, q.pm, f, (const C2<T>*)P->d_tw_c, work, st);
  }
  if (rc != NK_OK) return rc;
  if (hp.g.ndim == 3) {
    ProfScope ps(st, 6, f.pro, f.epi);
    rc = nk_dispatch_strided<T, 0>(hp.g.nm, q.s2, f, (const C2<T>*)P->d_tw_b, work, (C2<T>*)nullptr, st);
    if (rc != NK_OK) return rc;
  }
  if (!with_final) return NK_OK;
  ProfScope ps(st, 3, f.pro, f.epi);
  return nk_final_with_slots(hp, workspace, f, st, [&](const NkFuse& f2) {
    if (!C) return nk_dispatch_final3<T>(hp.g.nl, q.pf, f2, (const C2<T>*)P->d_tw_f, (const C2<T>*)work, st);
    for (int j = 0; j < C / 2; ++j) {
      NkPassF pf = q.pf;
      pf.a0 = j == 0 ? 0 : j * wc + 1;
      pf.a_cnt = (j + 1) * wc + 1 - pf.a0;
      int rcj = nk_dispatch_final3<T>(hp.g.nl, pf, f2, (const C2<T>*)P->d_tw_f, (const C2<T>*)work, st);
      if (rcj != NK_OK) return rcj;
      if (f.pipe_record) {
        hipError_t e = hipEventRecord((hipEvent_t)f.pipe_record[j], st);
        if (e != hipSuccess) return nk_set_hip_error(e, "hipEventRecord(pipe_record)");
      }
    }
    return (int)NK_OK;
  });
}

static int nk_sandwich_check(const nk_plan* P, const nk_fuse* fuse, int convention, void* workspace) {
  if (!P || !fuse) return nk_set_error(NK_ERR_INVALID, "nk_hartley_sandwich: null argument");
  if (!fuse->in || !fuse->out || !workspace) return nk_set_error(NK_ERR_INVALID, "nk_hartley_sandwich: in/out/workspace must be set");
  if (convention != NK_HARTLEY_NON_CANONICAL && convention != NK_HARTLEY_CANONICAL)
    return nk_set_error(NK_ERR_INVALID, "nk_hartley_sandwich: unknown hartley convention");
  if (!nk_plan_sandwich(P)) return nk_set_error(NK_ERR_UNSUPPORTED, "nk_hartley_sandwich: needs nk_plan_sandwich(plan) != 0");
  if (fuse->epi == NK_EPI_MUL)
    return nk_set_error(NK_ERR_INVALID, "nk_hartley_sandwich: `mul` is the diagonal between the transforms; the MUL epilogue is not available");
  if (fuse->cg_r && !(fuse->field_octant && fuse->pro == NK_PRO_AMP_JVP && fuse->dafield && fuse->cg_scal))
    return nk_set_error(NK_ERR_INVALID, "nk_hartley_sandwich: cg_r needs field_octant, the AMP_JVP prologue with dafield, and cg_scal");
  if ((fuse->pro == NK_PRO_AMP || fuse->pro == NK_PRO_AMP_JVP) && (!fuse->pidx || !fuse->amp))
    return nk_set_error(NK_ERR_INVALID, "nk_hartley_sandwich: AMP prologue needs pidx and amp");
  if (fuse->pro == NK_PRO_AMP_JVP && (!fuse->damp || !fuse->in2))
    return nk_set_error(NK_ERR_INVALID, "nk_hartley_sandwich: AMP_JVP prologue needs damp and in2");
  if (fuse->pro == NK_PRO_MUL && !fuse->in2) return nk_set_error(NK_ERR_INVALID, "nk_hartley_sandwich: MUL prologue needs in2");
  if (fuse->epi == NK_EPI_VJP && (!fuse->pidx || !fuse->amp || !fuse->xi || !fuse->abar))
    return nk_set_error(NK_ERR_INVALID, "nk_hartley_sandwich: VJP epilogue needs pidx, amp, xi and abar");
  if (fuse->epi == NK_EPI_LIKELIHOOD && (!fuse->data || !fuse->value))
    return nk_set_error(NK_ERR_INVALID, "nk_hartley_sandwich: LIKELIHOOD epilogue needs data and value");
  if (fuse->field_octant) {
    const bool amp_pro = fuse->pro == NK_PRO_AMP || fuse->pro == NK_PRO_AMP_JVP;
    if ((amp_pro && !fuse->afield) || (fuse->pro == NK_PRO_AMP_JVP && !fuse->dafield && !(fuse->pidx_octant && fuse->dampT)) ||
        (fuse->epi == NK_EPI_VJP && !fuse->afield))
      return nk_set_error(NK_ERR_INVALID, "nk_hartley_sandwich: field_octant needs afield (and dafield, or pidx_octant + dampT, for AMP_JVP)");
    const NkGeom& g = P->hp.g;
    if ((int64_t)(g.na / 2 + 1) * (g.nm / 2 + 1) * (g.nl / 2 + 1) >= ((int64_t)1 << 31))
      return nk_set_error(NK_ERR_UNSUPPORTED, "nk_hartley_sandwich: octant field too large (>= 2^31 elements)");
  }
  return NK_OK;
}

extern "C" int nk_hartley_sandwich(const nk_plan* P, const nk_fuse* fuse, double scale_first, int convention,
                                   void* workspace, void* stream) {
  const int rc = nk_sandwich_check(P, fuse, convention, workspace);
  if (rc != NK_OK) return rc;
  hipStream_t st = (hipStream_t)stream;
  if (P->hp.dtype == NK_F32) return nk_run_sandwich<float>(P, *fuse, scale_first, convention, workspace, st);
  return nk_run_sandwich<double>(P, *fuse, scale_first, convention, workspace, st);
}

template <typename T>
static int nk_run_sandwich_pair(const nk_plan* P, const NkFuse& fa, const NkFuse& fb, double scale_first, int convention,
                                void* wsa, void* wsb, hipStream_t st) {
  NkPipe3 q;
  int rc = nk_run_sandwich<T>(P, fa, scale_first, convention, wsa, st, false, &q);
  if (rc != NK_OK) return rc;
  rc = nk_run_sandwich<T>(P, fb, scale_first, convention, wsb, st, false, nullptr);
  if (rc != NK_OK) return rc;
  const NkHostPlan& hp = P->hp;
  ProfScope ps(st, 9, fa.pro, fa.epi);
  return nk_final_with_slots(hp, wsa, fa, st, [&](const NkFuse& fa2) {
    return nk_final_with_slots(hp, wsb, fb, st, [&](const NkFuse& fb2) {
      return nk_dispatch_final_pair<T>(hp.g.nl, q.pf, fa2, fb2, (const C2<T>*)P->d_tw_f, (const C2<T>*)wsa, (const C2<T>*)wsb, st);
    });
  });
}

extern "C" int nk_hartley_sandwich_pair(const nk_plan* P, const nk_fuse* fa, const nk_fuse* fb, double scale_first,
                                        int convention, void* workspace_a, void* workspace_b, void* stream) {
  int rc = nk_sandwich_check(P, fa, convention, workspace_a);
  if (rc != NK_OK) return rc;
  rc = nk_sandwich_check(P, fb, convention, workspace_b);
  if (rc != NK_OK) return rc;
  const bool vjp = fa->epi == NK_EPI_VJP && fb->epi == NK_EPI_VJP && fa->afield && fb->afield && fa->field_octant && fb->field_octant;
  if (!vjp || P->hp.g.ndim != 3 || fa->pipe_chunks || fb->pipe_chunks || workspace_a == workspace_b)
    return nk_set_error(NK_ERR_UNSUPPORTED, "nk_hartley_sandwich_pair: two VJP epilogues with octant amplitude fields on a 3-D plan, "
                                             "two workspaces, no slab pipelining");
  const bool joined = (fa->out == fb->out && fb->accumulate) || (fb->carry1 == fa->out && fb->out != fa->out);
  if (!joined || fa->w8 == fb->w8 || (fa->mul_scalar != fb->mul_scalar))
    return nk_set_error(NK_ERR_INVALID, "nk_hartley_sandwich_pair: B accumulates onto A's `out` or takes it as carry1; separate "
                                         "w8 areas, the same scalar diagonal");
  hipStream_t st = (hipStream_t)stream;
  if (P->hp.dtype == NK_F32) return nk_run_sandwich_pair<float>(P, *fa, *fb, scale_first, convention, workspace_a, workspace_b, st);
  return nk_run_sandwich_pair<double>(P, *fa, *fb, scale_first, convention, workspace_a, workspace_b, st);
}

extern "C" int nk_hartley(const nk_plan* P, const void* in, void* out, double scale, int convention, void* workspace,
                          void* stream) {
  nk_fuse f;
  memset(&f, 0, sizeof(f));
  f.pro = NK_PRO_PLAIN;
  f.in = in;
  f.epi = NK_EPI_AFFINE;
  f.out = out;
  f.scale = scale;
  f.offset = 0.0;
  return nk_hartley_fused(P, &f, convention, workspace, stream);
}

template <typename T>
static int nk_run_c2c(const nk_plan* P, const void* in, void* out, int inverse, double scale, hipStream_t st) {
  if (P->cc.lp.n == 0) return nk_set_error(NK_ERR_UNSUPPORTED, "nk_fftn: last axis too long for the c2c kernel");
  NkPassCC cc = P->cc;
  cc.swap = inverse ? 1 : 0;
  cc.scale = scale;
  const int64_t blocks = (cc.nlines + cc.tl.tile - 1) / cc.tl.tile;
  hipLaunchKernelGGL(k_c2c_contig<T>, dim3((unsigned)blocks), dim3(nk_gen_threads<T>(P->threads_cc)), P->lds_cc, st, cc,
                     (const C2<T>*)P->d_tw_cc, (const C2<T>*)in, (C2<T>*)out);
  int rc = nk_check_launch("k_c2c_contig");
  if (rc != NK_OK) return rc;
  if (P->ndim == 3) {
    const NkPassS& ps = P->c2c_mid;
    hipLaunchKernelGGL(k_c2c_strided<T>, dim3((unsigned)(ps.outer * ps.tiles_per_slab)), dim3(nk_gen_threads<T>(P->threads_cm)),
                       P->lds_cm, st, ps, cc.swap, (const C2<T>*)P->d_tw_b, (C2<T>*)out);
    rc = nk_check_launch("k_c2c_strided(mid)");
    if (rc != NK_OK) return rc;
  }
  if (P->ndim >= 2) {
    const NkPassS& ps = P->c2c_first;
    hipLaunchKernelGGL(k_c2c_strided<T>, dim3((unsigned)(ps.outer * ps.tiles_per_slab)), dim3(nk_gen_threads<T>(P->threads_cf)),
                       P->lds_cf, st, ps, cc.swap, (const C2<T>*)P->d_tw_c, (C2<T>*)out);
    rc = nk_check_launch("k_c2c_strided(first)");
  }
  return rc;
}

extern "C" int nk_fftn(const nk_plan* P, const void* in, void* out, int inverse, double scale, void* workspace,
                       void* stream) {
  (void)workspace;
  if (!P || !in || !out) return nk_set_error(NK_ERR_INVALID, "nk_fftn: null argument");
  hipStream_t st = (hipStream_t)stream;
  if (P->hp.dtype == NK_F32) return nk_run_c2c<float>(P, in, out, inverse, scale, st);
  return nk_run_c2c<double>(P, in, out, inverse, scale, st);
}
```

nifty_amd/csrc/nk_fft_batch.h:

```cpp
#pragma once
#include "nk_plan.h"
#include "nk_fft2.h"
#include "nk_util.h"

#ifndef NK_S0_WAVES
#define NK_S0_WAVES 1
#endif
#ifndef NK_PAIR_HAND_LDS_KB
#define NK_PAIR_HAND_LDS_KB 64
#endif
#ifndef NK_S1_TWO_WG
#define NK_S1_TWO_WG 0
#endif

template <typename T, bool COUPLES, int EC, int THREADS>
constexpr int nk_final_waves() {
  return THREADS > 256 ? 1 : (sizeof(T) == 8 && (COUPLES || EC == 2)) ? 2 : ((!COUPLES && sizeof(T) == 4 && (EC == 0 || EC == 1)) ? 4 : 3);
}

__device__ __forceinline__ void nk_flush_energy(const NkFuse& f, double acc, void* lds_raw) {
  if ((f.epi != NK_EPI_LIKELIHOOD && f.epi != NK_EPI_VJP) || f.value == nullptr) return;
  for (int off = 32; off > 0; off >>= 1) acc += __shfl_down(acc, off, 64);
  const int lane = threadIdx.x & 63, wave = threadIdx.x >> 6;
  const int nw = (blockDim.x + 63) >> 6;
  if (f.value_slots > 0) {
    const int64_t slot = (int64_t)blockIdx.x * nw + wave;
    if (lane == 0 && slot < f.value_slots) f.value[slot] = acc;
    return;
  }
  __syncthreads();
  double* red = (double*)lds_raw;
  if (lane == 0) red[wave] = acc;
  __syncthreads();
  if (threadIdx.x == 0) {
    double s = 0.0;
    for (int w = 0; w < nw; ++w) s += red[w];
    atomicAdd(f.value, s);
  }
}

__device__ __forceinline__ void nk_flush_wmax(const NkFuse& f, float wmax) {
#ifdef NK_WMAX_OFF
  return;
#endif
  if (f.w8max == nullptr || f.w8 == nullptr || f.epi != NK_EPI_VJP || f.value_slots <= 0) return;
  for (int off = 32; off > 0; off >>= 1) wmax = nk_wmax_join(wmax, __shfl_down(wmax, off, 64));
  const int lane = threadIdx.x & 63, wave = threadIdx.x >> 6;
  const int64_t slot = (int64_t)blockIdx.x * ((blockDim.x + 63) >> 6) + wave;
  if (lane == 0 && slot < f.value_slots) f.w8max[slot] = (double)wmax;
}


struct NkFuseArr {
  NkFuse f[NK_MAX_BATCH];
};
struct NkWorkArr {
  void* work[NK_MAX_BATCH];
  void* scratch[NK_MAX_BATCH];
};
struct NkBatchCtx {
  int count;
  const NkFuse* fuse;
  NkFuse final_fuse[NK_MAX_BATCH];
  NkWorkArr wa;
};
extern thread_local const NkBatchCtx* t_batch;
template <int N, int PC>
constexpr bool nk_twin_strided() {
  return N >= 512 && (PC == 0 || PC == 4 || PC == 5 || PC == 6);
}
template <int NL, bool COUPLES, int EC, int PAIR>
constexpr bool nk_twin_final() {
  return NL >= 512 && PAIR == 0 && ((COUPLES && EC == 2) || (!COUPLES && (EC == 1 || EC == 3 || EC == -1)) ||
                                    (!COUPLES && EC == 2 && NL >= 2048));
}

static bool nk_batch_class_ok(const NkGeom& g, const nk_fuse& f) {
  if (nk_knobs().ec_generic || g.na < 512 || g.nl < 512) return false;
  const bool pro_ok = f.pro == NK_PRO_PLAIN || f.pro == NK_PRO_MUL ||
                      (f.field_octant && !f.io32 && (f.pro == NK_PRO_AMP || f.pro == NK_PRO_AMP_JVP));
  const bool epi_ok = f.epi == NK_EPI_MUL || (f.epi == NK_EPI_LIKELIHOOD && !f.io32) || f.epi == NK_EPI_NONLIN ||
                      (f.epi == NK_EPI_VJP && f.afield);
  return pro_ok && epi_ok;
}


template <typename T, int N, int PC>
int nk_twin_launch_strided(const NkPassS& ps, int64_t blocks, const C2<T>* tw, int xmap, hipStream_t st);
template <typename T, int NL, bool COUPLES, int EC>
int nk_twin_launch_final(const NkPassF& pf, int64_t blocks, const C2<T>* tw, int xmap, hipStream_t st);

template <typename T>
int nk_tl_first_axis(const NkPassS& s1, int n1, int n2, const NkFuse& f, const C2<T>* tw_n1, const C2<T>* tw_n2, const C2<T>* tw_full,
                     C2<T>* work, hipStream_t st);

template <typename T, int NL>
int nk_launch_final_pair(NkPassF pf, const NkFuse& fa, const NkFuse& fb, const C2<T>* tw, const C2<T>* worka, const C2<T>* workb,
                         hipStream_t st);
```

nifty_amd/csrc/nk_plan.h:

```cpp
#pragma once
#include <cmath>
#include <cstdlib>
#include <vector>

#include "nk_fft_phases.h"

static inline NkLinePlan nk_make_line_plan(int n) {
  NkLinePlan lp{};
  lp.n = n;
  lp.nstage = 0;
  int rem = n;
  while (rem > 1) {
    int R;
    if (rem % 8 == 0) R = (rem == 16) ? 4 : 8;
    else if (rem % 4 == 0) R = 4;
    else if (rem % 2 == 0) R = 2;
    else if (rem % 3 == 0) R = 3;
    else if (rem % 5 == 0) R = 5;
    else if (rem % 7 == 0) R = 7;
    else {
      lp.nstage = -1;
      return lp;
    }
    if (lp.nstage == NK_MAX_STAGES) {
      lp.nstage = -1;
      return lp;
    }
    lp.radix[lp.nstage++] = R;
    rem /= R;
  }
  int span = n;
  for (int s = 0; s < lp.nstage; ++s) {
    span /= lp.radix[s];
    lp.span[s] = span;
    lp.dradix[s] = nk_make_div(lp.radix[s]);
    lp.dspan[s] = nk_make_div(span);
    lp.dnbf[s] = nk_make_div(n / lp.radix[s]);
  }
  return lp;
}
static inline bool nk_factorable(int64_t n) { return n >= 1 && n < ((int64_t)1 << 30) && nk_make_line_plan((int)n).nstage >= 0; }

static inline int nk_env_int(const char* name, int dflt) {
  const char* v = getenv(name);
  return v ? atoi(v) : dflt;
}

#ifndef NK_XMAP_DEFAULT
#define NK_XMAP_DEFAULT 9
#endif
struct NkKnobs {
  int fast = 1;
  int pipeline = 2;
  int xmap = NK_XMAP_DEFAULT;
  int work_blo = 0;
  int work_pad = 2080;
  int contig_quad = 1;
  int ec_generic = 0;
  int two_level = 1;
  int skip_final = 0;
  int mid_wg_per_cu = 0;
  int pair_hand = 0;
  int pair_pad_lds = 0;
  int tile_divides = 0;
};
static inline NkKnobs nk_read_knobs() {
  NkKnobs k;
  k.fast = nk_env_int("NK_FAST", k.fast);
  k.pipeline = nk_env_int("NK_PIPELINE", k.pipeline);
  k.xmap = nk_env_int("NK_XMAP", k.xmap);
  k.work_blo = nk_env_int("NK_WORK_BLO", k.work_blo);
  k.work_pad = nk_env_int("NK_WORK_PAD", k.work_pad);
  k.contig_quad = nk_env_int("NK_CONTIG_QUAD", k.contig_quad);
  k.ec_generic = nk_env_int("NK_EC_GENERIC", k.ec_generic);
  k.two_level = nk_env_int("NK_TWO_LEVEL", k.two_level);
  k.skip_final = nk_env_int("NK_SKIP_FINAL", k.skip_final);
  k.mid_wg_per_cu = nk_env_int("NK_MID_WG_PER_CU", k.mid_wg_per_cu);
  k.pair_hand = nk_env_int("NK_PAIR_HAND", k.pair_hand);
  k.pair_pad_lds = nk_env_int("NK_PAIR_PAD_LDS", k.pair_pad_lds);
  k.tile_divides = nk_env_int("NK_TILE_DIVIDES", k.tile_divides);
  return k;
}
inline NkKnobs nk_knobs() {
#ifdef NK_HOST_EMU
  return nk_read_knobs();
#else
  static const NkKnobs k = nk_read_knobs();
  return k;
#endif
}
static inline bool nk_contig3_quad(int64_t nblk, int ndim) {
  const int quad = nk_knobs().contig_quad;
  return (quad == 1 || (quad == 2 && nblk > 0)) && ndim == 3;
}

struct NkHostPlan {
  NkGeom g{};
  int dtype = 1;
  size_t csize = 16;
  NkPassA pa{};
  int threads_a = 256;
  size_t lds_a = 0;
  NkPassS pb{}, pc{};
  int threads_b = 256, threads_c = 256;
  size_t lds_b = 0, lds_c = 0;
  std::vector<double> tw_a, twr_a, tw_b, tw_c, tw_f;
  std::vector<double> tw_t64, tw_t32;
  size_t work_bytes = 0, scratch_bytes = 0;
};

static inline void nk_fill_twiddle(std::vector<double>& tw, int n, int denom) {
  tw.resize(2 * (size_t)(n > 0 ? n : 1));
  const long double w = -2.0L * 3.14159265358979323846264338327950288L / (long double)denom;
  for (int k = 0; k < n; ++k) {
    tw[2 * k] = (double)cosl(w * k);
    tw[2 * k + 1] = (double)sinl(w * k);
  }
  if (n <= 0) tw[0] = 1.0, tw[1] = 0.0;
}

static inline int nk_round_threads(int64_t work) {
  int64_t t = (work + 63) / 64 * 64;
  if (t < 64) t = 64;
  if (t > 1024) t = 1024;
  return (int)t;
}

static inline int nk_pick_strided_tile(int n, int64_t inner, size_t csize, const char* env, int64_t outer = 1 << 20) {
  int forced = nk_env_int(env, 0);
  size_t budget = 128 * 1024;
  int T = 1;
  const int divides = nk_knobs().tile_divides;
  auto fits = [&](int t) { return (int64_t)t <= inner && (!divides || inner % t == 0); };
  while (fits(T * 2) && (size_t)n * (T * 2) * csize <= budget && (size_t)(T * 2) * csize <= 256) T *= 2;
  if ((size_t)T * csize < 64) {
    budget = 152 * 1024;
    while (fits(T * 2) && (size_t)n * (T * 2) * csize <= budget && (size_t)(T * 2) * csize <= 256) T *= 2;
  }
  while (T > 4 && outer * ((inner + T - 1) / T) < 256) T /= 2;
  if (forced > 0) {
    T = 1;
    while (T * 2 <= forced && fits(T * 2) && (size_t)n * (T * 2) * csize <= 152 * 1024) T *= 2;
  }
  return T;
}

static inline int nk_host_plan_init(NkHostPlan& P, int ndim, const int64_t* shape, int dtype, int64_t batch,
                                    const char** msg) {
  *msg = "";
  if (ndim < 1 || ndim > 3) {
    *msg = "only 1, 2 or 3 transformed axes are supported";
    return NK_ERR_UNSUPPORTED;
  }
  if (dtype != NK_F32 && dtype != NK_F64) {
    *msg = "dtype must be NK_F32 or NK_F64";
    return NK_ERR_INVALID;
  }
  if (batch < 1) {
    *msg = "batch must be >= 1";
    return NK_ERR_INVALID;
  }
  for (int d = 0; d < ndim; ++d) {
    if (shape[d] < 1) {
      *msg = "axis lengths must be positive";
      return NK_ERR_INVALID;
    }
    if (!nk_factorable(shape[d])) {
      *msg = "axis lengths must factor into 2, 3, 5 and 7";
      return NK_ERR_UNSUPPORTED;
    }
  }
  if (shape[ndim - 1] < 2 || shape[ndim - 1] % 2 != 0) {
    *msg = "the last axis must have an even length >= 2 (real-to-complex packing)";
    return NK_ERR_UNSUPPORTED;
  }
  P.dtype = dtype;
  P.csize = dtype == NK_F32 ? 8 : 16;
  NkGeom& g = P.g;
  g.ndim = ndim;
  g.batch = (int)batch;
  g.nl = (int)shape[ndim - 1];
  g.h = g.nl / 2;
  g.na = ndim >= 2 ? (int)shape[0] : 1;
  g.nm = ndim == 3 ? (int)shape[1] : 1;
  g.sign = 1;
  const size_t max_line_bytes = 144 * 1024;
  if ((size_t)(g.h + g.h / 16 + 1) * P.csize > max_line_bytes || (size_t)g.na * P.csize > max_line_bytes ||
      (size_t)g.nm * P.csize > max_line_bytes) {
    *msg = "axis too long for a single-LDS line transform";
    return NK_ERR_UNSUPPORTED;
  }
  const int64_t n_total = batch * g.na * g.nm * g.nl;
  if (n_total >= ((int64_t)1 << 40)) {
    *msg = "array too large";
    return NK_ERR_UNSUPPORTED;
  }
  P.pa.g = g;
  P.pa.lp = nk_make_line_plan(g.h);
  P.pa.nlines = batch * g.na * g.nm;
  {
    const int lstride = g.h + g.h / 16 + 1;
    const size_t line_bytes = (size_t)lstride * P.csize;
    int64_t tile = (int64_t)(32 * 1024 / line_bytes);
    const int64_t want = (3072 + g.h - 1) / g.h;
    if (tile > want) tile = want;
    if (tile < 1) tile = 1;
    if (tile > P.pa.nlines) tile = P.pa.nlines;
    int forced = nk_env_int("NK_TILE_A", 0);
    if (forced > 0 && (size_t)forced * line_bytes <= 152 * 1024) tile = forced;
    P.pa.tl.tile = (int)tile;
    P.pa.tl.t_fastest = 0;
    P.pa.tl.tstride = 0;
    P.pa.tl.lstride = lstride;
    P.pa.tl.dtile = nk_make_div(tile);
    P.pa.dh = nk_make_div(g.h);
    P.pa.dnk = nk_make_div(g.h / 2 + 1);
    P.lds_a = (size_t)tile * line_bytes;
    P.threads_a = nk_round_threads(tile * g.h / 12);
    if (P.threads_a > 256) P.threads_a = 256;
    int ft = nk_env_int("NK_THREADS_A", 0);
    if (ft >= 64) P.threads_a = ft;
  }
  nk_fill_twiddle(P.tw_a, g.h, g.h);
  nk_fill_twiddle(P.twr_a, g.h / 2 + 1, g.nl);
  nk_fill_twiddle(P.tw_f, g.nl, g.nl);
  if (ndim == 2) nk_fill_twiddle(P.tw_t64, 64, 64), nk_fill_twiddle(P.tw_t32, 32, 32);
  auto setup_strided = [&](NkPassS& ps, int n, int64_t outer, int64_t inner, const char* env, int& threads,
                           size_t& lds, std::vector<double>& tw) {
    ps.g = g;
    ps.lp = nk_make_line_plan(n);
    ps.outer = outer;
    ps.inner = inner;
// ... 23 lines not shown
```

nifty_amd/engine.py:

```python
import contextlib
import ctypes
import math
import os
import threading

import numpy as np
import torch

from . import _lib as L
from . import backend as B
from . import batched, parallel, random
from .domains import PowerSpace, RGSpace
from .minimization import ConjugateGradient, Energy, QuadraticEnergy

SMALL_KEYS = ("asperity", "flexibility", "fluctuations", "loglogavgslope", "zeromode")
LATENT_KEYS = ("asperity", "flexibility", "fluctuations", "loglogavgslope", "spectrum", "xi", "zeromode")
_NONLIN = {None: L.NL_ID, "": L.NL_ID, "exp": L.NL_EXP, "sigmoid": L.NL_SIGMOID}
SPECTRUM_DEVICE_DRAW_MAX_POINTS = int(os.environ.get("NK_SPECTRUM_DEVICE_DRAW_MAX_POINTS", str(1 << 25)))


def lognormal_moments(mean, sigma):
    checked = {}
    for name, value in (("mean", mean), ("sig", sigma)):
        checked[name] = float(value)
# ... 738 lines not shown
            data, icov, wide = self._data64, self._icov64, torch.float64
        else:
            self._forward_nonlin(lp, x, self.tmp)
            mu = self.response.times(self.tmp)
            data, icov, wide = self.data, self.icov_field, self.tdtype
        if self.lh_kind == L.LH_GAUSS:
            r = B.axpby(1.0, mu, -1.0, data)
            ir = B.axpby(self.icov_scalar, r) if self.const_wd else B.binary(L.OP_MUL, r, icov)
            B.vdot(r, ir, result=lhval, accumulate=False)
            B.axpby(0.5, lhval, out=lhval)
        else:
            dat = self.data.to(wide)
            B.vsum(mu, result=lhval, accumulate=False)
            ld = B.vdot(B.pointwise("log", mu), dat)
            B.axpby(1.0, lhval, -1.0, ld, out=lhval)
            lp.wd = B.pointwise("reciprocal", mu)
            ir = B.binary(L.OP_SUB, 1.0, B.binary(L.OP_MUL, dat, lp.wd))
            lp.wd = lp.wd.to(self.tdtype)
        ir = ir.to(self.tdtype)
        if not want_gradient:
            return lp
        gs = self.response.adjoint(ir, self.shape)
        return self._finish_linearize(lp, x, gs, lp.gp, grad_acc, w, value, lhval)

    def _jvp_response(self, lp, d, cg_direction=None):
        L.check(L.load().nk_amp_jvp(self.nb, self.geo.data_ptr(), self.hyp.data_ptr(), lp.x.small.data_ptr(),
                                    lp.state.data_ptr(), d.small.data_ptr(), self.damp.data_ptr(), B._stream()), "nk_amp_jvp")
        self._amp_field(self.damp, out=self.dafield)
        f = self._fuse()
        f.pro, f.in_, f.in2 = L.PRO_AMP_JVP, d.xi.data_ptr(), lp.x.xi.data_ptr()
        f.pidx, f.amp, f.damp = self.pidx.data_ptr(), lp.amp.data_ptr(), self.damp.data_ptr()
        f.afield, f.dafield = B.ptr(lp.afield), self.dafield.data_ptr()
        f.epi, f.out, f.mul, f.mul_scalar = L.EPI_MUL, self.tmp.data_ptr(), lp.gp.data_ptr(), 1.0
        B.hartley_fused(self.plan, f)
        self._count("transforms", 1)
        return self.response.times(self.tmp)

    def lh_metric_accumulate(self, lp, d, out, scale, first, identity=0.0, dot_out=None, cg_direction=None, pipe=None,
                             addend=None, dest=None):
        if cg_direction is not None and not self.fused_direction:
            raise ValueError("cg_direction needs the sandwich pipeline (FusedModel.fused_direction)")
        if addend is not None and identity:
            raise ValueError("either the identity term or an explicit addend")
        avec, afac = (d, identity) if addend is None else addend
        if dest is None:
            dest = _Dest(out.xi, accumulate=not first)
        where = dict(accumulate=dest.accumulate, out_xi=dest.xi, carries=dest.carries)
        if self.response is not None:
            wsig = self.response.adjoint(self._weigh_data(self._jvp_response(lp, d), lp), self.shape)
            self._vjp(lp, wsig, scale, avec.xi if afac else None, afac, dot_out=dot_out, w2=lp.gp, **where)
            self._finish_metric(lp, avec, out, first, afac, dest)
            return
        L.check(L.load().nk_amp_jvp(self.nb, self.geo.data_ptr(), self.hyp.data_ptr(), lp.x.small.data_ptr(),
                                    lp.state.data_ptr(), d.small.data_ptr(), self.damp.data_ptr(), B._stream()), "nk_amp_jvp")
        gather_da = self.sandwich and self.pidx8 is not None and os.environ.get("NK_DA_GATHER", "0") == "1"
        if gather_da:
            damp_t = self.damp if self.tdtype == torch.float64 else self.damp.to(self.tdtype)
        else:
            self._amp_field(self.damp, out=self.dafield)

        def jvp_prologue(f):
            f.pro, f.in_, f.in2 = L.PRO_AMP_JVP, d.xi.data_ptr(), lp.x.xi.data_ptr()
            f.pidx, f.amp, f.damp = self.pidx.data_ptr(), lp.amp.data_ptr(), self.damp.data_ptr()
            f.afield = B.ptr(lp.afield)
            if gather_da:
                f.pidx_octant, f.dampT = self.pidx8.data_ptr(), damp_t.data_ptr()
            else:
                f.dafield = self.dafield.data_ptr()
            if cg_direction is not None:
                f.cg_r, f.cg_scal = cg_direction[0].xi.data_ptr(), cg_direction[1].scal.data_ptr()
            if pipe is not None:
                f.pipe_chunks = pipe[0]
                f.pipe_wait = None if pipe[1] is None else ctypes.cast(pipe[1], ctypes.c_void_p)
                f.pipe_record = None if pipe[2] is None else ctypes.cast(pipe[2], ctypes.c_void_p)

        if pipe is not None and not self.sandwich:
            raise ValueError("slab pipelining needs the sandwich pipeline")
        if self.sandwich:
            self._vjp(lp, None, scale, avec.xi if afac else None, afac, dot_out=dot_out,
                      sandwich=(jvp_prologue, self.h_dvol, lp.mid, lp.mid_scalar), **where)
            if cg_direction is not None:
                cg_direction[1].roll()
        else:
            f = self._fuse()
            jvp_prologue(f)
            f.epi, f.out, f.mul, f.mul_scalar = L.EPI_MUL, self.tmp.data_ptr(), B.ptr(lp.mid), lp.mid_scalar
            B.hartley_fused(self.plan, f)
            self._vjp(lp, self.tmp, scale, avec.xi if afac else None, afac, dot_out=dot_out, **where)
            self._count("transforms", 1)
        self._finish_metric(lp, avec, out, first, afac, dest)

    def pair_ready(self):
        return bool(self.sandwich and self.octant_vjp and self.response is None and self.bin_k2 is not None
                    and len(self.shape) == 3 and self.const_mid and os.environ.get("NK_PAIR_FINAL", "1") != "0")

    def _pair_buffers(self):
        if getattr(self, "_pair", None) is None:
            self._pair = dict(damp=torch.empty_like(self.damp), dafield=torch.empty_like(self.dafield),
                              w8=torch.empty_like(self.w8), w8max=torch.zeros_like(self.w8max),
                              workspace=torch.empty_like(self.plan.workspace))
        return self._pair

    def lh_metric_accumulate_pair(self, lpa, lpb, d, out, scale, first, identity=0.0, dot_out=None, cg_direction=None,
                                  dests=None, identity_first=0.0):
        if cg_direction is not None and not self.fused_direction:
            raise ValueError("cg_direction needs the sandwich pipeline (FusedModel.fused_direction)")
        pb = self._pair_buffers()
        lib = L.load()
        fuses = []
        if dests is None:
            dests = (_Dest(out.xi, accumulate=not first), _Dest(out.xi, accumulate=True))
        for lp, damp, dafield, w8, w8max, dest in ((lpa, self.damp, self.dafield, self.w8, self.w8max, dests[0]),
                                                   (lpb, pb["damp"], pb["dafield"], pb["w8"], pb["w8max"], dests[1])):
            L.check(lib.nk_amp_jvp(self.nb, self.geo.data_ptr(), self.hyp.data_ptr(), lp.x.small.data_ptr(), lp.state.data_ptr(),
                                   d.small.data_ptr(), damp.data_ptr(), B._stream()), "nk_amp_jvp")
            self._amp_field(damp, out=dafield)
            f = self._fuse()
            f.pro, f.in_, f.in2 = L.PRO_AMP_JVP, d.xi.data_ptr(), lp.x.xi.data_ptr()
            f.pidx, f.amp, f.damp = self.pidx.data_ptr(), lp.amp.data_ptr(), damp.data_ptr()
            f.afield, f.dafield = B.ptr(lp.afield), dafield.data_ptr()
            f.mul, f.mul_scalar = B.ptr(lp.mid), lp.mid_scalar
            f.epi, f.out, f.scale = L.EPI_VJP, dest.xi.data_ptr(), self.h_dvol * scale
            f.xi = lp.x.xi.data_ptr()
            f.addend, f.addend_scale, f.accumulate = None, 0.0, 1 if dest.accumulate else 0
            f.carry1, f.carry2 = (B.ptr(c) for c in (tuple(dest.carries) + (None, None))[:2])
            f.abar, f.w8 = self.abar.data_ptr(), w8.data_ptr()
            if self.scatter_fixed_point:
                f.w8max = w8max.data_ptr()
            fuses.append(f)
        if cg_direction is not None:
            fuses[0].cg_r, fuses[0].cg_scal = cg_direction[0].xi.data_ptr(), cg_direction[1].scal.data_ptr()
        if identity_first:
            fuses[0].addend, fuses[0].addend_scale = d.xi.data_ptr(), identity_first
        if identity:
            fuses[1].addend, fuses[1].addend_scale = d.xi.data_ptr(), identity
            if dot_out is not None:
                fuses[1].value = dot_out.data_ptr()
        elif dot_out is not None:
            raise ValueError("dot_out needs the identity term (the addend of the epilogue)")
        B.hartley_sandwich_pair(self.plan, fuses[0], fuses[1], self.h_dvol, pb["workspace"])
        _PairTree.settle(dests[1])
        if cg_direction is not None:
            cg_direction[1].roll()
        self._count("transforms", 4)
        shp = (ctypes.c_int64 * len(self.shape))(*self.shape)
        for lp, w8, w8max, is_first, dest, ident in ((lpa, self.w8, self.w8max, first, dests[0], identity_first),
                                                     (lpb, pb["w8"], pb["w8max"], False, dests[1], identity)):
            L.check(lib.nk_octant_scatter_k2(len(self.shape), shp, w8.data_ptr(), self.pidx.data_ptr(), self.bin_k2.data_ptr(),
                                             self.nb, self.scatter_scratch.data_ptr(), self.abar.data_ptr(),
                                             w8max.data_ptr() if self.scatter_fixed_point else 0, B._stream()),
                    "nk_octant_scatter_k2")
            self._finish_metric(lp, d, out, is_first, ident, dest)

    def _finish_metric(self, lp, d, out, first, identity, dest=None):
        self._amp_vjp(lp)
        if dest is not None:
            _PairTree.settle(dest)
            if dest.small is not None:
                dest.small.append(B.axpby(1.0, self.latbar, identity, d.small) if identity else B.axpby(1.0, self.latbar))
                self._count("metric", 1)
                return
        if first:
            out.small = B.axpby(1.0, self.latbar, identity, d.small) if identity else B.axpby(1.0, self.latbar)
        else:
            B.axpby(1.0, self.latbar, 1.0, out.small, out=out.small)
            if identity:
                B.axpby(identity, d.small, 1.0, out.small, out=out.small)
        self._count("metric", 1)

    def metric(self, lp, d, dot_out=None, cg_direction=None):
        out = LatentVec(torch.empty_like(d.xi), None)
        self.lh_metric_accumulate(lp, d, out, 1.0, True, identity=1.0, dot_out=dot_out, cg_direction=cg_direction)
        return out

    def lh_metric(self, lp, d, minus=None):
        out = LatentVec(torch.empty_like(d.xi), None)
        self.lh_metric_accumulate(lp, d, out, 1.0, True, addend=None if minus is None else (minus, -1.0))
        return out

    def trafo_point(self, x):
        lp = LinPoint()
        lp.x = x
        lp.amp, lp.state = self._amp_forward(x.small)
        lp.afield = self._amp_field(lp.amp)
        if self.response is not None:
            self._forward_nonlin(lp, x, self.tmp)
            mu = self.response.times(self.tmp)
            if self.lh_kind == L.LH_GAUSS:
                lp.tfd = math.sqrt(self.icov_scalar) if self.icov_field is None else B.pointwise("sqrt", self.icov_field)
                lp.f = B.axpby(lp.tfd, mu) if self.icov_field is None else B.binary(L.OP_MUL, mu, lp.tfd)
            else:
                rt = B.pointwise("sqrt", mu)
                lp.f, lp.tfd = B.axpby(2.0, rt), B.pointwise("reciprocal", rt)
            return lp
        f = self._fuse()
        f.pro, f.in_, f.pidx, f.amp = L.PRO_AMP, x.xi.data_ptr(), self.pidx.data_ptr(), lp.amp.data_ptr()
        f.afield = lp.afield.data_ptr()
        g = torch.empty(self.shape, dtype=self.tdtype, device=self.device)
        gp = torch.empty_like(g)
        f.epi, f.out, f.out2, f.offset, f.nonlin = L.EPI_NONLIN, g.data_ptr(), gp.data_ptr(), self.offset_mean, self.nonlin
        B.hartley_fused(self.plan, f)
        self._count("transforms", 1)
        if self.lh_kind == L.LH_GAUSS:
            if self.icov_field is None:
                tw = math.sqrt(self.icov_scalar)
                lp.f, lp.tf = B.axpby(tw, g), B.axpby(tw, gp)
            else:
                tw = B.pointwise("sqrt", self.icov_field)
                lp.f, lp.tf = B.binary(L.OP_MUL, g, tw), B.binary(L.OP_MUL, gp, tw)
        else:
            rt = B.pointwise("sqrt", g)
            lp.f, lp.tf = B.axpby(2.0, rt), B.binary(L.OP_DIV, gp, rt)
        return lp

    def jvp_data(self, lp, d, out=None):
        if self.response is not None:
            u = self._jvp_response(lp, d)
            return B.axpby(lp.tfd, u, out=out) if np.isscalar(lp.tfd) else B.binary(L.OP_MUL, u, lp.tfd, out=out)
        L.check(L.load().nk_amp_jvp(self.nb, self.geo.data_ptr(), self.hyp.data_ptr(), lp.x.small.data_ptr(),
                                    lp.state.data_ptr(), d.small.data_ptr(), self.damp.data_ptr(), B._stream()), "nk_amp_jvp")
        f = self._fuse()
        f.pro, f.in_, f.in2 = L.PRO_AMP_JVP, d.xi.data_ptr(), lp.x.xi.data_ptr()
        f.pidx, f.amp, f.damp = self.pidx.data_ptr(), lp.amp.data_ptr(), self.damp.data_ptr()
        f.afield = B.ptr(lp.afield)
        self._amp_field(self.damp, out=self.dafield)
        f.dafield = self.dafield.data_ptr()
        out = torch.empty(self.shape, dtype=self.tdtype, device=self.device) if out is None else out
        f.epi, f.out, f.mul, f.mul_scalar = L.EPI_MUL, out.data_ptr(), lp.tf.data_ptr(), 1.0
        B.hartley_fused(self.plan, f)
        self._count("transforms", 1)
        return out

    def vjp_data(self, lp, w, addend=None):
        out = LatentVec(torch.empty_like(lp.x.xi), None)
        w2 = lp.tf
        if self.response is not None:
            u = B.axpby(lp.tfd, w) if np.isscalar(lp.tfd) else B.binary(L.OP_MUL, w, lp.tfd)
            w, w2 = self.response.adjoint(u, self.shape), lp.gp
        self._vjp(lp, w, 1.0, None if addend is None else addend.xi, 1.0, False, out.xi, w2=w2)
        self._amp_vjp(lp)
        out.small = B.axpby(1.0, self.latbar) if addend is None else B.axpby(1.0, self.latbar, 1.0, addend.small)
        return out

    def _upload(self, arr, dtype):
        return torch.from_numpy(np.ascontiguousarray(arr)).to(dtype).to(self.device)

    def host_draws_before_xi(self, sseq):
        rng = np.random.default_rng(sseq)
        fresh = rng.bit_generator.state
        vals = {}
        for k in LATENT_KEYS:
            if k == "xi":
                break
            vals[k] = rng.normal(0.0, 1.0, (2, self.nb - 2) if k == "spectrum" else ())
        return vals, rng.bit_generator.state, fresh

    def draw_prior(self, device_rng=None, ahead=None):
        if device_rng is not None:
            xi = torch.randn(self.shape, dtype=self.tdtype, device=self.device, generator=device_rng)
            small = torch.randn(self.nsmall, dtype=torch.float64, device=self.device, generator=device_rng)
            return LatentVec(xi, small)
        nb = self.nb
        parts = {}
        if ahead is not None:
            if random.current_rng().bit_generator.state != ahead[2]:
                raise RuntimeError("draw_prior(ahead=...): the random context has advanced since its seed was handed to the "
                                   "draw-ahead worker")
            random.current_rng().bit_generator.state = ahead[1]
        for k in LATENT_KEYS:
            if ahead is not None and k in ahead[0]:
                if k == "spectrum":
                    spectrum = self._upload(ahead[0][k], torch.float64)
                else:
                    parts[k] = ahead[0][k]
                continue
            if k == "xi":
                xi = random.Random.normal_on_device(self.npdtype, self.shape, 0.0, 1.0, self.device)
            elif k == "spectrum":
                if self.N <= SPECTRUM_DEVICE_DRAW_MAX_POINTS:
                    spectrum = random.Random.normal_on_device(np.float64, (2, nb - 2), 0.0, 1.0, self.device)
                else:
                    spectrum = self._upload(random.current_rng().normal(0.0, 1.0, (2, nb - 2)), torch.float64)
            else:
                parts[k] = random.current_rng().normal(0.0, 1.0, ())
        small = torch.empty(self.nsmall, dtype=torch.float64, device=self.device)
        small[:5].copy_(torch.from_numpy(np.array([parts[k] for k in SMALL_KEYS], dtype=np.float64)), non_blocking=False)
        small[5:].copy_(spectrum.reshape(-1))
        return LatentVec(xi, small)

    def draw_lh_noise(self, lp, device_rng=None):
        if self.response is not None:
            dshape = self.data_shape
            if device_rng is not None:
                eta = torch.randn(dshape, dtype=self.tdtype, device=self.device, generator=device_rng)
                if self.const_wd:
                    eta = B.axpby(math.sqrt(self.icov_scalar), eta)
            else:
                eta = random.Random.normal_on_device(self.npdtype, dshape, 0.0,
                                                     math.sqrt(self.icov_scalar) if self.const_wd else 1.0, self.device)
            if not self.const_wd:
                eta = B.binary(L.OP_MUL, eta, B.pointwise("sqrt", self.icov_field if self.lh_kind == L.LH_GAUSS else lp.wd))
            out = LatentVec(torch.empty(self.shape, dtype=self.tdtype, device=self.device), None)
            self._vjp(lp, self.response.adjoint(eta, self.shape), 1.0, None, 0.0, False, out.xi, w2=lp.gp)
            self._amp_vjp(lp)
            out.small = B.axpby(1.0, self.latbar)
            return out
# ... 372 lines not shown
                                 torch.empty_like(shard_vec.small))
        full = out_full.xi.reshape(-1).view(self.chunks, -1)
        mine = shard_vec.xi.view(self.chunks, self.m)
        for c in range(self.chunks):
            self.comm.all_gather(mine[c], full[c])
        out_full.small.copy_(shard_vec.small)
        return out_full

    def apply(self, d_full):
        staged = self.chunks > 1 and self.overlap
        timer = parallel.exchange_timer
        with timer.span("local_metric"):
            out = self.kl._apply_metric_local(d_full, pipe=(self.chunks, None, None) if staged else None)
        with timer.span("exposed_wait"), timer.span("reduce_scatter"):
            return self._reduce(out)

    def _scatter_chunk(self, full_chunk, share):
        if self.kl._across:
            self.comm.tree_reduce_slices(full_chunk, share)
        else:
            self.comm.reduce_scatter_sum(full_chunk, share)

    def _sum_small(self, small):
        if self.kl._across:
            self.comm.tree_allreduce_gathered_([small])
        else:
            self.comm.allreduce_sum_([small])

    def _reduce(self, out):
        q_xi = torch.empty(self.chunks * self.m, dtype=out.xi.dtype, device=out.xi.device)
        full = out.xi.reshape(-1).view(self.chunks, -1)
        for c in range(self.chunks):
            self._scatter_chunk(full[c], q_xi[c * self.m:(c + 1) * self.m])
        self._sum_small(out.small)
        return LatentVec(q_xi, out.small)

    def apply_shard(self, d_shard, d_full):
        timer = parallel.exchange_timer
        P, nbytes = self.comm.size, d_full.xi.numel() * d_full.xi.element_size()
        timer.count(2 * (P - 1) * nbytes // P)
        if self._side is None:
            with timer.span("iteration"):
                with timer.span("exposed_wait"), timer.span("all_gather"):
                    self.gather(d_shard, d_full)
                return self.apply(d_full)
        cur = torch.cuda.current_stream(self.model.device)
        side, pairs = self._side, self._stage_chunks()
        full = d_full.xi.reshape(-1).view(self.chunks, -1)
        mine = d_shard.xi.view(self.chunks, self.m)
        with timer.span("iteration", cur):
            d_full.small.copy_(d_shard.small)
            side.wait_stream(cur)
            with torch.cuda.stream(side), timer.span("all_gather", side):
                for j, pair in enumerate(pairs):
                    for c in pair:
                        self.comm.all_gather(mine[c], full[c])
                    self._ev_in[j].record(side)
            with timer.span("local_metric", cur):
                out = self.kl._apply_metric_local(d_full, pipe=(self.chunks, self._h_in, self._h_out))
            q_xi = torch.empty(self.chunks * self.m, dtype=out.xi.dtype, device=out.xi.device)
            ofull = out.xi.reshape(-1).view(self.chunks, -1)
            with torch.cuda.stream(side):
                for j, pair in enumerate(pairs):
                    side.wait_event(self._ev_out[j])
                    with timer.span("reduce_scatter", side):
                        for c in pair:
                            self._scatter_chunk(ofull[c], q_xi[c * self.m:(c + 1) * self.m])
            with timer.span("exposed_wait", cur):
                cur.wait_stream(side)
            self._sum_small(out.small)
        return LatentVec(q_xi, out.small)


class FusedGeoEnergy(Energy):

    def __init__(self, model, tp_p, m, position, nanisinf=True):
        super().__init__(position)
        self.model, self.tp_p, self.m = model, tp_p, m
        self.tp = model.trafo_point(position)
        gx = model.vjp_data(tp_p, self.tp.f, addend=position)
        self.res = gx - m
        val = 0.5 * self.res.s_vdot(self.res)
        self._value = math.inf if (math.isnan(val) and nanisinf) else val
        self._grad = self._G_T(self.res)

    def _G(self, d):
        return self.model.vjp_data(self.tp_p, self.model.jvp_data(self.tp, d), addend=d)

    def _G_T(self, y):
        return self.model.vjp_data(self.tp, self.model.jvp_data(self.tp_p, y), addend=y)

    @property
    def value(self):
        return self._value

    @property
    def gradient(self):
        return self._grad

    def at(self, position):
        return FusedGeoEnergy(self.model, self.tp_p, self.m, position)

    def apply_metric(self, d):
        return self._G_T(self._G(d))

    @property
    def metric(self):
        return _Callable(self.apply_metric)


def share_range(nwork, nshares, myshare):
    return parallel.shareRange(nwork, nshares, myshare)


def draw_samples(model, position, n_samples, mirror_samples, controller_factory, comm=None, device_rng=None,
                 geo_minimizer=None):
    plan = parallel.SamplePlan(n_samples, mirror_samples, comm)
    plan.check_synchronised()
    cache = {}

    def linearisation():
        if "lp" not in cache:
            cache["lp"] = model.metric_point(position)
        return cache["lp"]

    drawn_seeds = [plan.seeds[i] for i in range(plan.lo, plan.hi) if not (plan.mirror and i % 2 == 1 and i > plan.lo)]
    ahead = None
    want_ahead = (device_rng is None and model.N > SPECTRUM_DEVICE_DRAW_MAX_POINTS and bool(drawn_seeds)
                  and os.environ.get("NK_DRAW_AHEAD", "1") != "0")

    def draw(seed):
        if device_rng is not None:
            device_rng.manual_seed(int(seed.generate_state(1, np.uint64)[0] >> np.uint64(1)))
        lp = linearisation()
        return model.draw_mgvi_sample(lp, controller_factory(), device_rng, ahead=ahead.take(seed) if ahead else None)

    def linear_residual(pair, mirrored):
        return pair[1], mirrored

    def fitted_residual(pair, mirrored):
        if "tp" not in cache:
            cache["tp"] = model.trafo_point(position)
            cache["g_p"] = model.vjp_data(cache["tp"], cache["tp"].f, addend=position)
        b, y = pair
        target = cache["g_p"] - b if mirrored else cache["g_p"] + b
        start = position - y if mirrored else position + y
        fit, _ = geo_minimizer(FusedGeoEnergy(model, cache["tp"], target, start))
        return fit.position - position, False

    finish = linear_residual if geo_minimizer is None else fitted_residual
    local_pairs = len({i // 2 if plan.mirror else i for i in range(plan.lo, plan.hi)})
    lanes = _sampling_lanes(model, local_pairs)
    in_batch = local_pairs >= 2 and batched.ready(model)
    if lanes is None and not in_batch:
        if want_ahead:
            ahead = _HostDrawAhead(model, drawn_seeds)
        try:
            drawn = plan.run(draw, finish)
        finally:
            if ahead is not None:
                ahead.close()
    else:
        together = geo_minimizer is not None and lanes is not None and os.environ.get("NK_GEO_THREADS", "1") != "0"
        if in_batch:
            solve = lambda jobs: batched.solve_together(model, linearisation(), jobs, controller_factory)
        else:
            solve = lambda jobs: _solve_on_lanes(model, lanes, linearisation(), jobs, controller_factory)
        drawn = plan.run_together(lambda seed: _draw_sources(model, linearisation(), seed, device_rng), solve,
                                  (lambda pair, mirrored: (pair, mirrored)) if together else finish)
        if together:
            if "tp" not in cache:
                cache["tp"] = model.trafo_point(position)
                cache["g_p"] = model.vjp_data(cache["tp"], cache["tp"].f, addend=position)
            fits = _fit_on_lanes(model, lanes, cache["tp"], cache["g_p"], position, drawn, geo_minimizer)
            drawn = [(f, False) for f in fits]
    return [r for r, _ in drawn], [n for _, n in drawn], plan.n_total


class _HostDrawAhead:

    def __init__(self, model, seeds):
        from concurrent.futures import ThreadPoolExecutor

        self._model, self._seeds = model, list(seeds)
        self._pool = ThreadPoolExecutor(max_workers=1)
        self._pending = {}
        self._start(0)

    def _start(self, k):
        if k < len(self._seeds):
            self._pending[k] = self._pool.submit(self._model.host_draws_before_xi, self._seeds[k])

    def take(self, seed):
        k = next((j for j, sq in enumerate(self._seeds) if sq is seed), None)
        fut = self._pending.pop(k, None) if k is not None else None
        if k is not None:
            self._start(k + 1)
        if k is not None and k + 1 >= len(self._seeds):
            self._pool.shutdown(wait=False)
        return fut.result() if fut is not None else None

    def close(self):
        self._pending.clear()
        self._pool.shutdown(wait=False, cancel_futures=True)


def _fit_on_lanes(model, lanes, tp, g_p, position, jobs, minimizer):
    import copy
    from concurrent.futures import ThreadPoolExecutor

    main = torch.cuda.current_stream(model.device)
    K = min(len(lanes), len(jobs))
    points = []
    for _ in range(K):
        own = copy.copy(tp)
        own.state = tp.state.clone()
        points.append(own)
    for lane in lanes[1:K]:
        lane.stream.wait_stream(main)
    out = [None] * len(jobs)

    def work(k):
        lane, mine = lanes[k], copy.deepcopy(minimizer)
        torch.cuda.set_device(model.device)
        with torch.cuda.stream(lane.stream if lane.stream is not None else main):
            for j in range(k, len(jobs), K):
                (b, y), mirrored = jobs[j]
                target = g_p - b if mirrored else g_p + b
                start = position - y if mirrored else position + y
                fit, _ = mine(FusedGeoEnergy(lane, points[k], target, start))
                out[j] = fit.position - position

    with ThreadPoolExecutor(max_workers=K) as pool:
        list(pool.map(work, range(K)))
    for lane in lanes[1:K]:
        main.wait_stream(lane.stream)
    for r in out:
        r.xi.record_stream(main)
        r.small.record_stream(main)
    return out


def _sampling_lanes(model, pairs):
    want = int(os.environ.get("NK_LANES", "4"))
    small = model.N <= int(os.environ.get("NK_LANE_MAX_POINTS", str(1 << 25)))
    if want < 2 or pairs < 2 or not small or (model.response is not None and os.environ.get("NK_LANES_RESPONSE", "1") == "0"):
        return None
    return model.lanes(min(want, pairs))


def _draw_sources(model, lp, seed, device_rng):
    if device_rng is not None:
        device_rng.manual_seed(int(seed.generate_state(1, np.uint64)[0] >> np.uint64(1)))
    return model.draw_prior(device_rng), model.draw_lh_noise(lp, device_rng)


def _solve_on_lanes(model, lanes, lp, jobs, controller_factory):
    import copy

    main = torch.cuda.current_stream(model.device)
    pairs = []
    points = []
    for lane in lanes:
        own = copy.copy(lp)
        own.state = lp.state.clone()
        points.append(own)
    for w0 in range(0, len(jobs), len(lanes)):
        wave = jobs[w0:w0 + len(lanes)]
        problems = []
        for lane, lp, (s, nj) in zip(lanes, points, wave):
            if lane.stream is not None:
                lane.stream.wait_stream(main)
            with (torch.cuda.stream(lane.stream) if lane.stream is not None else contextlib.nullcontext()):
                b = s + nj
                g0 = lane.lh_metric(lp, s, minus=nj)
                A = _Callable(lambda v, dot_out=None, cg_direction=None, lane=lane, lp=lp: lane.metric(lp, v, dot_out=dot_out,
                                                                                                       cg_direction=cg_direction),
                              fused_dot=lane.octant_vjp, fused_direction=lane.fused_direction)
                energy = QuadraticEnergy(s, A, b, _grad=g0)
                energy.consumable = True
            controller = controller_factory()
            if any(controller is other[1] for other in problems):
                controller = copy.deepcopy(controller)
            problems.append((energy, controller, lane.stream, b))
        solved = ConjugateGradient(None).solve_many([p[:3] for p in problems])
        for (energy, _), (_, _, stream, b) in zip(solved, problems):
            if stream is not None:
                main.wait_stream(stream)
                for t in (b.xi, b.small, energy.position.xi, energy.position.small):
                    t.record_stream(main)
            pairs.append((b, energy.position))
    return pairs


def mgvi_iteration(model, mean, n_samples, controller_factory, kl_minimizer, mirror_samples=True, comm=None,
                   device_rng=None, geo_minimizer=None, on_phase=None):
    residuals, negs, n_total = draw_samples(model, mean, n_samples, mirror_samples, controller_factory, comm, device_rng,
                                            geo_minimizer)
    if on_phase is not None:
        on_phase("sampling")
    kl = FusedKL(model, mean, residuals, negs, n_total, comm)
    if on_phase is not None:
        on_phase("kl_construction")
    with parallel.lockstep(comm):
        kl, _ = kl_minimizer(kl)
    if on_phase is not None:
        on_phase("newton_cg")
    return kl.position, kl
```

nifty_amd/minimization.py:

```python
import functools
import logging
from time import time

import numpy as np

logger = logging.getLogger("nifty_amd")

CONVERGED, CONTINUE, ERROR = 0, 1, 2
class _Counters(dict):

    def __init__(self, *a, **kw):
        import threading

        super().__init__(*a, **kw)
        self._lock = threading.Lock()

    def add(self, key, n=1):
        with self._lock:
            self[key] += n


counters = _Counters(cg_iterations=0)


# ... 312 lines not shown
    import os

    return os.environ.get("NK_CG_ENERGY_RECURRENCE", "1") != "0"


class _ScalarEnergyView:

    def __init__(self, value, gradnorm):
        self.value, self.gradient_norm = value, gradnorm


class _HostCg:

    def __init__(self, energy, preconditioner, refresh_every):
        self.energy, self._precondition = energy, (lambda v: v) if preconditioner is None else preconditioner
        self._refresh_every, self._since_refresh = refresh_every, 0
        self.r = energy.gradient
        self.d = self._precondition(self.r)
        self.gamma = None

    @staticmethod
    def _dot(u, v):
        return _ls(np.real(u.s_vdot(v)))

    def _bad(self, what):
        logger.error(f"ConjugateGradient stops: {what}")
        return ERROR

    def begin(self):
        self.gamma = self._dot(self.r, self.d)
        if np.isnan(self.gamma):
            return self._bad("the first <r, P r> is not a number")
        return CONVERGED if self.gamma == 0 else None

    def iterate(self, controller):
        q = self.energy.apply_metric(self.d)
        counters.add("cg_iterations")
        curvature = self._dot(self.d, q)
        if np.isnan(curvature) or curvature == 0.0:
            return self._bad("the curvature <d, A d> is zero or not a number")
        step = self.gamma / curvature
        if step < 0:
            return self._bad("negative step length: the operator is not positive definite along the search direction")
        where = self.energy.position - step * self.d
        self._since_refresh += 1
        if self._since_refresh < self._refresh_every:
            self.r = self.r - q * step
            self.energy = self.energy.at_with_grad(where, self.r)
        else:
            self.energy = self.energy.at(where)
            self.r, self._since_refresh = self.energy.gradient, 0
        s = self._precondition(self.r)
        gamma = self._dot(self.r, s)
        if np.isnan(gamma):
            return self._bad("<r, P r> is not a number")
        if gamma < 0:
            return self._bad("<r, P r> < 0: the preconditioner is not positive definite")
        if gamma == 0:
            return CONVERGED
        _lockstep_flush()
        status = controller.check(self.energy)
        if status != CONTINUE:
            return status
        self.d = self.d * max(0, gamma / self.gamma) + s
        self.gamma = gamma
        return None


CG_NRESET = 20


class ConjugateGradient(Minimizer):

    def __init__(self, controller, nreset=None):
        nreset = CG_NRESET if nreset is None else nreset
        self._controller = controller
        self._nreset = nreset

    def __call__(self, energy, preconditioner=None):
        if preconditioner is None and hasattr(energy.position, "cg_workspace") and isinstance(energy, QuadraticEnergy):
            return self._solve_inplace(energy)
        return self._solve_generic(energy, preconditioner)

    def _solve_generic(self, energy, preconditioner):
        status = self._controller.start(energy)
        if status != CONTINUE:
            return energy, status
        cg = _HostCg(energy, preconditioner, self._nreset)
        status = cg.begin()
        while status is None:
            status = cg.iterate(self._controller)
        return cg.energy, status

    def _solve_inplace(self, energy):
        A, b = energy._A, energy._b
        sm = getattr(A, "sharded", None)
        if sm is not None and b is not None:
            status = self._controller.start(energy)
            if status != CONTINUE:
                return energy, status
            return self._solve_inplace_sharded(energy, sm)
        steps = self._inplace_steps(energy, self._controller)
        while True:
            try:
                next(steps)
            except StopIteration as done:
                return done.value

    def solve_many(self, problems):
        import contextlib

        import torch

        runs = [self._inplace_steps(energy, controller) for energy, controller, _ in problems]
        results, active = [None] * len(problems), list(range(len(problems)))
        while active:
            for k in list(active):
                stream = problems[k][2]
                with (torch.cuda.stream(stream) if stream is not None else contextlib.nullcontext()):
                    try:
                        next(runs[k])
                    except StopIteration as done:
                        results[k] = done.value
                        active.remove(k)
        return results

    def _inplace_steps(self, energy, controller):
        status = controller.start(energy)
        if status != CONTINUE:
            return energy, status
        A, b = energy._A, energy._b
        if getattr(energy, "consumable", False):
            x, r = energy.position, energy.gradient
        else:
            x, r = energy.position.clone(), energy.gradient.clone()
        d = r.clone()
        ws = x.cg_workspace()
        gamma_prev = _ls(r.s_vdot(r))
        if np.isnan(gamma_prev):
            return energy, ERROR
        if gamma_prev == 0:
            return energy, CONVERGED
        ws.set_gamma(gamma_prev)
        since_reset = 0

        def finish(status):
            return energy.at_with_grad(x, r), status

        track_energy = hasattr(ws, "update_dr") and _config_track_energy()
        value = float(energy.value) if track_energy else None
        fused_dot = bool(getattr(A, "fused_dot", False)) and hasattr(ws, "curv_slot")
        fused_dir = bool(getattr(A, "fused_direction", False)) and hasattr(ws, "direction_small")

        def device_iteration(with_direction):
            extra = {}
            if with_direction and fused_dir:
                ws.direction_small(d, r)
                extra["cg_direction"] = (r, ws)
            elif with_direction:
                ws.direction(d, r)
            if fused_dot:
                q = A(d, dot_out=ws.curv_slot(), **extra)
                ws.curv_small(d, q)
            else:
                q = A(d, **extra)
                ws.curv(d, q)
            if track_energy:
                ws.update_dr(x, r, d, q)
            else:
                ws.update(x, r, d, q, b)

        ahead = hasattr(ws, "fetch_begin") and not fused_dir
        direction_done = False
        iteration = 0
        while True:
            iteration += 1
            device_iteration(iteration > 1 and not direction_done)
            direction_done = False
            counters.add("cg_iterations")
            since_reset += 1
            refreshed = False
            if since_reset >= self._nreset and not _forced_stop(controller):
                Ax = A(x)
                r = Ax - b if b is not None else Ax
                ws.refresh(x, r, b)
                since_reset = 0
                refreshed = True
            if ahead:
                ws.fetch_begin()
                ws.direction(d, r)
                direction_done = True
            yield
            sc = ws.fetch_end() if ahead else ws.fetch()
            curv, gamma, alpha = sc["curv"], sc["gamma"], sc["alpha"]
            if np.isnan(curv) or curv == 0.0 or np.isnan(alpha) or alpha < 0:
                logger.error("Error: ConjugateGradient: bad curvature / step")
                return finish(ERROR)
            if np.isnan(gamma) or gamma < 0:
                return finish(ERROR)
            if gamma == 0:
                return finish(CONVERGED)
            if track_energy and not refreshed:
                value = value - alpha * sc["dr"] + 0.5 * alpha * alpha * curv
            else:
                value = 0.5 * sc["xr"] - 0.5 * sc["xb"] if b is not None else 0.5 * sc["xr"]
            status = controller.check(_ScalarEnergyView(value, float(np.sqrt(gamma))))
            if status != CONTINUE:
                return finish(status)


    def _solve_inplace_sharded(self, energy, sm):
        controller = self._controller
        b_full = energy._b
        b = sm.shard(b_full)
        x = sm.shard(energy.position, copy=True)
        r = sm.shard(energy.gradient, copy=True)
        d = r.clone()
        d_full = energy.gradient.clone()
        ws = sm.workspace()
        track_energy = hasattr(ws, "update_dr") and _config_track_energy()
        value = float(energy.value) if track_energy else None
        gamma_prev = float(ws.dot(r, r, 0).item())
        if np.isnan(gamma_prev):
            return energy, ERROR
        if gamma_prev == 0:
            return energy, CONVERGED
        since_reset = 0

        def finish(status):
            return energy.at_with_grad(sm.gather(x), sm.gather(r)), status

        while True:
            q = sm.apply_shard(d, d_full)
            ws.curv(d, q)
            if track_energy:
                ws.update_dr(x, r, d, q)
            else:
                ws.update(x, r, d, q, b)
            counters.add("cg_iterations")
            since_reset += 1
            refreshed = False
            if since_reset >= self._nreset and not _forced_stop(controller):
                Ax = sm.apply(sm.gather(x))
                r = Ax - b
                ws.refresh(x, r, b)
                since_reset = 0
                refreshed = True
            sc = ws.fetch()
            curv, gamma, alpha = sc["curv"], sc["gamma"], sc["alpha"]
            if np.isnan(curv) or curv == 0.0 or np.isnan(alpha) or alpha < 0:
                logger.error("Error: ConjugateGradient: bad curvature / step")
                return finish(ERROR)
            if np.isnan(gamma) or gamma < 0:
                return finish(ERROR)
            if gamma == 0:
                return finish(CONVERGED)
            if track_energy and not refreshed:
                value = value - alpha * sc["dr"] + 0.5 * alpha * alpha * curv
            else:
                value = 0.5 * sc["xr"] - 0.5 * sc["xb"]
            status = controller.check(_ScalarEnergyView(value, float(np.sqrt(gamma))))
            if status != CONTINUE:
                return finish(status)
            ws.direction(d, r)


class LineEnergy:

    def __init__(self, line_position, energy, line_direction, offset=0.0):
        self._t = float(line_position)
        self._dir = line_direction
        if self._t == float(offset):
            self._energy = energy
        else:
            self._energy = energy.at(position=energy.position + (self._t - float(offset)) * self._dir)

    def at(self, line_position):
        return LineEnergy(line_position, self._energy, self._dir, offset=self._t)

    @property
    def energy(self):
        return self._energy

    @property
    def value(self):
        return self._energy.value

    @property
    def directional_derivative(self):
        return _ls(np.real(self._energy.gradient.s_vdot(self._dir)))


def _interp_cubic(a, fa, fpa, b, fb, c, fc):
    with np.errstate(divide="raise", over="raise", invalid="raise"):
        try:
            db, dc = b - a, c - a
            denom = (db * dc) ** 2 * (db - dc)
            m = np.array([[dc * dc, -db * db], [-dc ** 3, db ** 3]])
            A, B = m @ np.array([fb - fa - fpa * db, fc - fa - fpa * dc])
            A, B = A / denom, B / denom
            xmin = a + (-B + np.sqrt(B * B - 3 * A * fpa)) / (3 * A)
        except ArithmeticError:
            return None
    return xmin if np.isfinite(xmin) else None


def _interp_quadratic(a, fa, fpa, b, fb):
    with np.errstate(divide="raise", over="raise", invalid="raise"):
        try:
            db = b - a * 1.0
            B = (fb - fa - fpa * db) / (db * db)
            xmin = a - fpa / (2.0 * B)
        except ArithmeticError:
            return None
    return xmin if np.isfinite(xmin) else None


class _Wolfe:

    def __init__(self, phi0, dphi0, c1, c2):
        self.phi0, self.dphi0, self._c1, self._c2 = phi0, dphi0, c1, c2

    def too_high(self, t, phi):
        return phi > self.phi0 + self._c1 * t * self.dphi0

    def flat_enough(self, dphi):
        return abs(dphi) <= -self._c2 * self.dphi0


class LineSearch:

    def __init__(self, preferred_initial_step_size=None, c1=1e-4, c2=0.9, max_step_size=1e30, max_iterations=100,
                 max_zoom_iterations=100):
        self.preferred_initial_step_size = preferred_initial_step_size
        self.c1, self.c2 = float(c1), float(c2)
        self.max_step_size = max_step_size
# ... 320 lines not shown
```

Before: 0.2130.

## Group up to four CG sample solves into shared Hartley sandwich launches

Adds a grouped Hartley sandwich entry point that runs the first contiguous pass and the final pass for up to four independent metric applications in one kernel launch each. Blocks are interleaved across members in chunks of eight. The sampling driver gains a grouped path that steps several conjugate-gradient solves as generators and flushes their metric applications together. This fills the GPU better and amortizes launches on large grids, at the cost of per-member workspaces, extra memory pressure and a more complex scheduling path.

```diff
diff --git a/include/niftyk.h b/include/niftyk.h
--- a/include/niftyk.h
+++ b/include/niftyk.h
@@ -87,6 +87,11 @@
                         void* stream);
 int nk_hartley_sandwich_pair(const nk_plan* plan, const nk_fuse* fuse_a, const nk_fuse* fuse_b, double scale_first,
                              int convention, void* workspace_a, void* workspace_b, void* stream);
+#define NK_MAX_GROUP 4
+int nk_hartley_sandwich_group(const nk_plan* plan, const nk_fuse* fuses, int count, double scale_first, int convention,
+                              void* const* workspaces, void* stream);
+int nk_group_order(int64_t bid, int count, int64_t* member, int64_t* local);
+int64_t nk_group_grid_size(int64_t per, int count);
 int nk_fftn(const nk_plan* plan, const void* in, void* out, int inverse, double scale, void* workspace,
             void* stream);
 
diff --git a/nifty_amd/_lib.py b/nifty_amd/_lib.py
--- a/nifty_amd/_lib.py
+++ b/nifty_amd/_lib.py
@@ -61,6 +61,9 @@
     "nk_plan_pipe_ok": (_i, [_vp, _i]),
     "nk_hartley_sandwich": (_i, [_vp, ctypes.POINTER(Fuse), _d, _i, _vp, _vp]),
     "nk_hartley_sandwich_pair": (_i, [_vp, ctypes.POINTER(Fuse), ctypes.POINTER(Fuse), _d, _i, _vp, _vp, _vp]),
+    "nk_hartley_sandwich_group": (_i, [_vp, ctypes.POINTER(Fuse), _i, _d, _i, _vp, _vp]),
+    "nk_group_order": (_i, [_i64, _i, ctypes.POINTER(_i64), ctypes.POINTER(_i64)]),
+    "nk_group_grid_size": (_i64, [_i64, _i]),
     "nk_fftn": (_i, [_vp, _vp, _vp, _i, _d, _vp, _vp]),
     "nk_profile_enable": (_i, [_i]),
     "nk_profile_collect": (_i, [_vp, _vp]),
@@ -135,6 +138,7 @@
     "nk_cg_direction_batch": (_i, [_i64, _i, _vp, _vp, _i, _vp, _i, _vp]),
 }
 MAX_BATCH = 8
+MAX_GROUP = 4
 
 
 def ptr_array(tensors):
diff --git a/nifty_amd/backend.py b/nifty_amd/backend.py
--- a/nifty_amd/backend.py
+++ b/nifty_amd/backend.py
@@ -258,6 +258,15 @@
     L.check(L.load().nk_hartley_sandwich_pair(plan.handle, ctypes.byref(fuse_a), ctypes.byref(fuse_b), float(scale_first),
                                               _convention(), plan.workspace.data_ptr(), workspace_b.data_ptr(), _stream()),
             "nk_hartley_sandwich_pair")
+
+
+def hartley_sandwich_group(plan, fuses, scale_first, workspaces):
+    if plan.device.index != _current_device():
+        _wrong_device(plan.device.index)
+    arr = (L.Fuse * len(fuses))(*fuses)
+    L.check(L.load().nk_hartley_sandwich_group(plan.handle, arr, len(fuses), float(scale_first), _convention(),
+                                               ctypes.cast(L.ptr_array(workspaces), ctypes.c_void_p), _stream()),
+            "nk_hartley_sandwich_group")
 
 
 def fftn(x, ndim=None, inverse=False, scale=1.0):
@@ -781,7 +790,7 @@
     return wrapper
 
 
-for _name in ("cplx_rows", "cplx_pointwise", "hartley", "hartley_fused", "hartley_sandwich", "hartley_sandwich_pair", "fftn", "vdot", "vsum", "binary", "axpby",
+for _name in ("cplx_rows", "cplx_pointwise", "hartley", "hartley_fused", "hartley_sandwich", "hartley_sandwich_pair", "hartley_sandwich_group", "fftn", "vdot", "vsum", "binary", "axpby",
               "axpby_sqnorm",
               "pointwise", "gather", "scatter_add", "bin_plan", "bin_sum", "spmv", "spmv_t", "stats", "cumsum"):
     globals()[_name] = _runs_on_operand_device(globals()[_name])
diff --git a/nifty_amd/csrc/nk_fft.hip b/nifty_amd/csrc/nk_fft.hip
--- a/nifty_amd/csrc/nk_fft.hip
+++ b/nifty_amd/csrc/nk_fft.hip
@@ -301,22 +301,6 @@
   nk_contig3_body<T, H, Contig3Tile<T, H>::TILE, PC>(ex, p, f, blockIdx.x, (T*)smem, tw, twr, work);
 }
 
-#ifndef NK_QUAD_MAXW_F64_5
-#define NK_QUAD_MAXW_F64_5 4
-#endif
-#ifndef NK_QUAD_MAXW_F64_8
-#define NK_QUAD_MAXW_F64_8 8
-#endif
-#ifndef NK_QUAD_MAXW_F32_5
-#define NK_QUAD_MAXW_F32_5 8
-#endif
-#ifndef NK_QUAD_MAXW_F32_8
-#define NK_QUAD_MAXW_F32_8 8
-#endif
-template <typename T, int PC>
-constexpr int nk_quad_max_waves() {
-  return sizeof(T) == 8 ? (PC == 8 ? NK_QUAD_MAXW_F64_8 : NK_QUAD_MAXW_F64_5) : (PC == 8 ? NK_QUAD_MAXW_F32_8 : NK_QUAD_MAXW_F32_5);
-}
 template <typename T, int H, int PC>
 __global__ void __launch_bounds__((Contig3Tile<T, H>::QTHREADS))
     k3_contig_quad(NkPass3 p, NkFuse f, const C2<T>* __restrict__ tw, const C2<T>* __restrict__ twr, C2<T>* __restrict__ work) {
@@ -1166,7 +1150,7 @@
 
 template <typename T>
 static int nk_run_sandwich(const nk_plan* P, const NkFuse& f, double scale_first, int convention, void* workspace, hipStream_t st,
-                           bool with_final = true, NkPipe3* q_out = nullptr) {
+                           bool with_final = true, NkPipe3* q_out = nullptr, bool with_first = true) {
   const NkHostPlan& hp = P->hp;
   const int sign = convention == NK_HARTLEY_CANONICAL ? -1 : 1;
   const int work_pad = nk_knobs().work_pad;
@@ -1186,7 +1170,9 @@
                                                "the first axis, and an octant amplitude prologue");
   }
   const int wc = C ? hp.g.na / C : 0;
-  if (C) {
+  if (!with_first) {
+    if (C) return nk_set_error(NK_ERR_UNSUPPORTED, "grouped first pass: no slab pipelining");
+  } else if (C) {
     const int Mh = hp.g.nm / 2 + 1;
     for (int j = 0; j < C / 2; ++j) {
       if (f.pipe_wait) {
@@ -1280,13 +1266,177 @@
   return nk_run_sandwich<double>(P, *fuse, scale_first, convention, workspace, st);
 }
 
+
+extern "C" int nk_group_order(int64_t bid, int count, int64_t* member, int64_t* local) {
+  if (bid < 0 || count < 1 || count > NK_MAX_GROUP || !member || !local)
+    return nk_set_error(NK_ERR_INVALID, "nk_group_order: bid >= 0, 1 <= count <= NK_MAX_GROUP");
+  nk_group_decode(bid, count, *member, *local);
+  return NK_OK;
+}
+extern "C" int64_t nk_group_grid_size(int64_t per, int count) { return nk_group_grid(per, count); }
+
+static bool nk_group_first_ok(const nk_plan* P, const nk_fuse* fuses, int count) {
+  const NkGeom& g = P->hp.g;
+  if (!nk_knobs().group || g.ndim != 3 || g.batch != 1 || !nk_contig3_quad(0, 3)) return false;
+  if (!(P->hp.dtype == NK_F32 ? nk_contig3_quad_ok<float>(g.h) : nk_contig3_quad_ok<double>(g.h))) return false;
+  for (int m = 0; m < count; ++m) {
+    const nk_fuse& f = fuses[m];
+    if (!(f.field_octant && f.pro == NK_PRO_AMP_JVP && f.dafield) || f.pipe_chunks || !f.cg_r != !fuses[0].cg_r) return false;
+  }
+  return true;
+}
+static bool nk_group_final_ok(const nk_plan* P, const nk_fuse* fuses, int count) {
+  const NkGeom& g = P->hp.g;
+  if (!nk_knobs().group || g.ndim != 3 || g.batch != 1 || nk_knobs().skip_final) return false;
+  for (int m = 0; m < count; ++m)
+    if (!(fuses[m].epi == NK_EPI_VJP && fuses[m].afield && fuses[m].field_octant) || fuses[m].pipe_chunks) return false;
+  return true;
+}
+
+template <typename T>
+static int nk_group_first(const nk_plan* P, const NkPass3& p1, const nk_fuse* fuses, int count, void* const* ws, hipStream_t st) {
+  NkGroupFuse fa;
+  NkGroupWork wa;
+  for (int m = 0; m < NK_MAX_GROUP; ++m) {
+    fa.f[m] = fuses[m < count ? m : 0];
+    wa.work[m] = ws[m < count ? m : 0];
+  }
+  const bool c8 = fuses[0].cg_r != nullptr;
+  ProfScope ps(st, 5, c8 ? 4 : fuses[0].pro, fuses[0].epi, count);
+  const C2<T>* tw = (const C2<T>*)P->d_tw_a;
+  const C2<T>* twr = (const C2<T>*)P->d_twr_a;
+  return nk_dispatch_fast(P->hp.g.h, "no fast contiguous pass for this length", [&](auto N) {
+    return c8 ? nk_group_launch_contig3<T, N(), 8>(p1, fa, wa, count, tw, twr, st) : nk_group_launch_contig3<T, N(), 5>(p1, fa, wa, count, tw, twr, st);
+  });
+}
+
+template <typename T>
+static int nk_group_final(const nk_plan* P, const NkPassF& pf, const nk_fuse* fuses, int count, void* const* ws, hipStream_t st, int m,
+                          NkGroupFuse& fa) {
+  const NkHostPlan& hp = P->hp;
+  if (m < count)
+    return nk_final_with_slots(hp, ws[m], fuses[m], st, [&](const NkFuse& f2) {
+      fa.f[m] = f2;
+      return nk_group_final<T>(P, pf, fuses, count, ws, st, m + 1, fa);
+    });
+  NkGroupWork wa;
+  for (int k = 0; k < NK_MAX_GROUP; ++k) {
+    if (k >= count) fa.f[k] = fa.f[0];
+    wa.work[k] = ws[k < count ? k : 0];
+  }
+  return nk_dispatch_fast(hp.g.nl, "no fast final pass for this length",
+                          [&](auto N) { return nk_group_launch_final<T, N()>(pf, fa, wa, count, (const C2<T>*)P->d_tw_f, st); });
+}
+
+template <typename T>
+static int nk_run_sandwich_group(const nk_plan* P, const nk_fuse* fuses, int count, double scale_first, int convention, void* const* ws,
+                                 hipStream_t st) {
+  const bool gfirst = nk_group_first_ok(P, fuses, count), gfinal = nk_group_final_ok(P, fuses, count);
+  if (count == 1 || (!gfirst && !gfinal)) {
+    for (int m = 0; m < count; ++m) {
+      const int rc = nk_run_sandwich<T>(P, fuses[m], scale_first, convention, ws[m], st);
+      if (rc != NK_OK) return rc;
+    }
+    return NK_OK;
+  }
+  const NkHostPlan& hp = P->hp;
+  const NkPipe3 q = nk_pipe3_setup<T>(hp, convention == NK_HARTLEY_CANONICAL ? -1 : 1, nk_knobs().work_pad, 1.0);
+  if (nk_pipe3_work_elems(hp.g, nk_pipe3_colpad<T>(), nk_knobs().work_pad) * sizeof(C2<T>) > hp.work_bytes)
+    return nk_set_error(NK_ERR_RUNTIME, "nk_hartley_sandwich: plan workspace too small");
+  int rc;
+  if (gfirst) {
+    rc = nk_group_first<T>(P, q.p1, fuses, count, ws, st);
+    if (rc != NK_OK) return rc;
+  }
+  for (int m = 0; m < count; ++m) {
+    rc = nk_run_sandwich<T>(P, fuses[m], scale_first, convention, ws[m], st, !gfinal, nullptr, !gfirst);
+    if (rc != NK_OK) return rc;
+  }
+  if (!gfinal) return NK_OK;
+  NkGroupFuse fa;
+  ProfScope ps(st, 3, fuses[0].pro, fuses[0].epi, count);
+  return nk_group_final<T>(P, q.pf, fuses, count, ws, st, 0, fa);
+}
+
+struct NkSpan {
+  const char* lo;
+  const char* hi;
+  bool written;
+};
+static int nk_member_spans(const nk_plan* P, const nk_fuse& f, void* workspace, NkSpan* out) {
+  const NkGeom& g = P->hp.g;
+  const size_t ts = P->hp.dtype == NK_F32 ? 4 : 8;
+  const size_t full = (size_t)g.batch * g.na * g.nm * g.nl * ts;
+  const size_t oct_n = (size_t)(g.na / 2 + 1) * (g.nm / 2 + 1) * (g.nl / 2 + 1);
+  int n = 0;
+  auto add = [&](const void* p, size_t bytes, bool written) {
+    if (p) out[n++] = NkSpan{(const char*)p, (const char*)p + bytes, written};
+  };
+  add(f.in, full, f.cg_r != nullptr);
+  add(f.in2, full, false);
+  add(f.cg_r, full, false);
+  add(f.xi, full, false);
+  add(f.addend, full, false);
+  add(f.carry1, full, false);
+  add(f.carry2, full, false);
+  add(f.mul, full, false);
+  add(f.afield, f.field_octant ? oct_n * ts : full, false);
+  add(f.dafield, f.field_octant ? oct_n * ts : full, false);
+  add(f.out, full, true);
+  add(f.w8, (size_t)g.batch * oct_n * sizeof(double), true);
+  add(f.w8max, sizeof(double), true);
+  add(f.value, sizeof(double), true);
+  if (!f.w8 && f.abar) add(f.abar, (size_t)((f.abar_copies > 1 ? f.abar_copies - 1 : 0) * f.abar_stride + 1) * sizeof(double), true);
+  add(workspace, nk_plan_workspace_bytes(P), true);
+  return n;
+}
+
+extern "C" int nk_hartley_sandwich_group(const nk_plan* P, const nk_fuse* fuses, int count, double scale_first, int convention,
+                                         void* const* workspaces, void* stream) {
+  if (!P || !fuses || !workspaces || count < 1 || count > NK_MAX_GROUP)
+    return nk_set_error(NK_ERR_INVALID, "nk_hartley_sandwich_group: bad argument (1 <= count <= NK_MAX_GROUP)");
+  if (P->hp.g.ndim != 3) return nk_set_error(NK_ERR_UNSUPPORTED, "nk_hartley_sandwich_group: 3-D plans only");
+  NkSpan spans[NK_MAX_GROUP][20];
+  int nspan[NK_MAX_GROUP];
+  for (int m = 0; m < count; ++m) {
+    const int rc = nk_sandwich_check(P, fuses + m, convention, workspaces[m]);
+    if (rc != NK_OK) return rc;
+    if (fuses[m].pipe_chunks) return nk_set_error(NK_ERR_UNSUPPORTED, "nk_hartley_sandwich_group: no slab pipelining");
+    if (!nk_same_class(fuses[0], fuses[m]) || !fuses[0].cg_r != !fuses[m].cg_r)
+      return nk_set_error(NK_ERR_INVALID, "nk_hartley_sandwich_group: the members select different kernel classes");
+    nspan[m] = nk_member_spans(P, fuses[m], workspaces[m], spans[m]);
+    for (int k = 0; k < m; ++k)
+      for (int i = 0; i < nspan[m]; ++i)
+        for (int j = 0; j < nspan[k]; ++j) {
+          const NkSpan &a = spans[m][i], &b = spans[k][j];
+          if ((a.written || b.written) && a.lo < b.hi && b.lo < a.hi)
+            return nk_set_error(NK_ERR_INVALID, "nk_hartley_sandwich_group: an array one member writes overlaps an array of another "
+                                                 "member (in under cg_r, out, w8, w8max, value, abar and the workspace are written)");
+        }
+  }
+  hipStream_t st = (hipStream_t)stream;
+  if (P->hp.dtype == NK_F32) return nk_run_sandwich_group<float>(P, fuses, count, scale_first, convention, workspaces, st);
+  return nk_run_sandwich_group<double>(P, fuses, count, scale_first, convention, workspaces, st);
+}
+
 template <typename T>
 static int nk_run_sandwich_pair(const nk_plan* P, const NkFuse& fa, const NkFuse& fb, double scale_first, int convention,
                                 void* wsa, void* wsb, hipStream_t st) {
   NkPipe3 q;
-  int rc = nk_run_sandwich<T>(P, fa, scale_first, convention, wsa, st, false, &q);
+  int rc;
+  const nk_fuse pair[2] = {fa, fb};
+  void* const wsp[2] = {wsa, wsb};
+  const bool gfirst = !fa.cg_r && !fb.cg_r && nk_same_class(fa, fb) && nk_group_first_ok(P, pair, 2);
+  if (gfirst) {
+    const NkPipe3 q0 = nk_pipe3_setup<T>(P->hp, convention == NK_HARTLEY_CANONICAL ? -1 : 1, nk_knobs().work_pad, 1.0);
+    if (nk_pipe3_work_elems(P->hp.g, nk_pipe3_colpad<T>(), nk_knobs().work_pad) * sizeof(C2<T>) > P->hp.work_bytes)
+      return nk_set_error(NK_ERR_RUNTIME, "nk_hartley_sandwich: plan workspace too small");
+    rc = nk_group_first<T>(P, q0.p1, pair, 2, wsp, st);
+    if (rc != NK_OK) return rc;
+  }
+  rc = nk_run_sandwich<T>(P, fa, scale_first, convention, wsa, st, false, &q, !gfirst);
   if (rc != NK_OK) return rc;
-  rc = nk_run_sandwich<T>(P, fb, scale_first, convention, wsb, st, false, nullptr);
+  rc = nk_run_sandwich<T>(P, fb, scale_first, convention, wsb, st, false, nullptr, !gfirst);
   if (rc != NK_OK) return rc;
   const NkHostPlan& hp = P->hp;
   ProfScope ps(st, 9, fa.pro, fa.epi);
diff --git a/nifty_amd/csrc/nk_fft_batch.h b/nifty_amd/csrc/nk_fft_batch.h
--- a/nifty_amd/csrc/nk_fft_batch.h
+++ b/nifty_amd/csrc/nk_fft_batch.h
@@ -97,3 +97,44 @@
 template <typename T, int NL>
 int nk_launch_final_pair(NkPassF pf, const NkFuse& fa, const NkFuse& fb, const C2<T>* tw, const C2<T>* worka, const C2<T>* workb,
                          hipStream_t st);
+
+NK_HD void nk_group_decode(int64_t bid, int count, int64_t& member, int64_t& local) {
+  const int64_t span = 8 * (int64_t)count;
+  const int64_t g = bid / span, w = bid % span;
+  member = w / 8;
+  local = 8 * g + w % 8;
+}
+static inline int64_t nk_group_grid(int64_t per, int count) { return (per + 7) / 8 * 8 * count; }
+struct NkGroupFuse {
+  NkFuse f[NK_MAX_GROUP];
+};
+struct NkGroupWork {
+  void* work[NK_MAX_GROUP];
+};
+
+#ifndef NK_QUAD_MAXW_F64_5
+#define NK_QUAD_MAXW_F64_5 4
+#endif
+#ifndef NK_QUAD_MAXW_F64_8
+#define NK_QUAD_MAXW_F64_8 8
+#endif
+#ifndef NK_QUAD_MAXW_F32_5
+#define NK_QUAD_MAXW_F32_5 8
+#endif
+#ifndef NK_QUAD_MAXW_F32_8
+#define NK_QUAD_MAXW_F32_8 8
+#endif
+template <typename T, int PC>
+constexpr int nk_quad_max_waves() {
+  return sizeof(T) == 8 ? (PC == 8 ? NK_QUAD_MAXW_F64_8 : NK_QUAD_MAXW_F64_5) : (PC == 8 ? NK_QUAD_MAXW_F32_8 : NK_QUAD_MAXW_F32_5);
+}
+
+template <typename T, int H, int PC>
+int nk_group_launch_contig3(const NkPass3& p3, const NkGroupFuse& fa, const NkGroupWork& wa, int count, const C2<T>* tw, const C2<T>* twr,
+                            hipStream_t st);
+template <typename T, int NL>
+int nk_group_launch_final(NkPassF pf, const NkGroupFuse& fa, const NkGroupWork& wa, int count, const C2<T>* tw, hipStream_t st);
+template <typename T, int H>
+constexpr bool nk_group_quad_ok() {
+  return Contig3Tile<T, H>::QUAD_OK;
+}
diff --git a/nifty_amd/csrc/nk_fft_g.hip b/nifty_amd/csrc/nk_fft_g.hip
--- /dev/null
+++ b/nifty_amd/csrc/nk_fft_g.hip
@@ -0,0 +1,115 @@
+#include <hip/hip_runtime.h>
+
+#include "nk_fft_batch.h"
+
+template <typename T, int H, int PC>
+__device__ __forceinline__ void nk_group_contig3(const NkPass3& p, const NkGroupFuse& fa, const NkGroupWork& wa, int count, int64_t per,
+                                                 const C2<T>* __restrict__ tw, const C2<T>* __restrict__ twr, unsigned char* smem) {
+  int64_t member, local;
+  nk_group_decode((int64_t)blockIdx.x, count, member, local);
+  if (local >= per) return;
+  DeviceExec<T, Contig3Tile<T, H>::SC::E> ex;
+  nk_contig3_body<T, H, 4, PC, true>(ex, p, fa.f[member], local, (T*)smem, tw, twr, (C2<T>*)wa.work[member], 0);
+}
+template <typename T, int H, int PC>
+__global__ void __launch_bounds__((Contig3Tile<T, H>::QTHREADS))
+    k3_contig_quad_g(NkPass3 p, NkGroupFuse fa, NkGroupWork wa, int count, int64_t per, const C2<T>* __restrict__ tw,
+                     const C2<T>* __restrict__ twr) {
+  extern __shared__ __align__(16) unsigned char smem[];
+  nk_group_contig3<T, H, PC>(p, fa, wa, count, per, tw, twr, smem);
+}
+template <typename T, int H, int PC, int MAXW>
+__global__ void __launch_bounds__((Contig3Tile<T, H>::QTHREADS)) __attribute__((amdgpu_waves_per_eu(1, MAXW)))
+    k3_contig_quad_gw(NkPass3 p, NkGroupFuse fa, NkGroupWork wa, int count, int64_t per, const C2<T>* __restrict__ tw,
+                      const C2<T>* __restrict__ twr) {
+  extern __shared__ __align__(16) unsigned char smem[];
+  nk_group_contig3<T, H, PC>(p, fa, wa, count, per, tw, twr, smem);
+}
+template <typename T, int H, int PC>
+static constexpr auto nk_group_quad_kernel() {
+  if constexpr (nk_quad_max_waves<T, PC>() < 8)
+    return k3_contig_quad_gw<T, H, PC, nk_quad_max_waves<T, PC>()>;
+  else
+    return k3_contig_quad_g<T, H, PC>;
+}
+
+template <typename T, int H, int PC>
+int nk_group_launch_contig3(const NkPass3& p3, const NkGroupFuse& fa, const NkGroupWork& wa, int count, const C2<T>* tw, const C2<T>* twr,
+                            hipStream_t st) {
+  using CT = Contig3Tile<T, H>;
+  if constexpr (!CT::QUAD_OK) {
+    return nk_set_error(NK_ERR_UNSUPPORTED, "grouped first pass: no QUAD build for this length");
+  } else {
+    const int64_t per = (int64_t)(p3.g.na / 2 + 1) * (p3.g.nm / 2 + 1);
+    const int64_t grid = nk_group_grid(per, count);
+    if (p3.nblk > 0 || p3.nlines != (int64_t)p3.g.na * p3.g.nm || grid > 0x7fffffffLL)
+      return nk_set_error(NK_ERR_UNSUPPORTED, "grouped first pass: one unstaged grid per member");
+    NkPass3 pq = p3;
+    pq.blk0 = 0;
+    pq.dmh = nk_make_div(p3.g.nm / 2 + 1);
+    return nk_launch<nk_group_quad_kernel<T, H, PC>()>("k3_contig_quad_g", dim3((unsigned)grid), dim3(CT::QTHREADS), CT::QLDS_BYTES, st, pq, fa,
+                                                       wa, count, per, tw, twr);
+  }
+}
+
+__device__ __forceinline__ void nk_group_flush(const NkFuse& f, double acc, float wmax, int64_t local) {
+  const int lane = threadIdx.x & 63, wave = threadIdx.x >> 6;
+  const int64_t slot = local * ((blockDim.x + 63) >> 6) + wave;
+  if (f.value != nullptr && f.value_slots > 0) {
+    for (int off = 32; off > 0; off >>= 1) acc += __shfl_down(acc, off, 64);
+    if (lane == 0 && slot < f.value_slots) f.value[slot] = acc;
+  }
+#ifndef NK_WMAX_OFF
+  if (f.w8max != nullptr && f.w8 != nullptr && f.value_slots > 0) {
+    for (int off = 32; off > 0; off >>= 1) wmax = nk_wmax_join(wmax, __shfl_down(wmax, off, 64));
+    if (lane == 0 && slot < f.value_slots) f.w8max[slot] = (double)wmax;
+  }
+#endif
+}
+
+template <typename T, int NL>
+__global__ void __launch_bounds__((FinalTile<T, NL, 2, 2>::THREADS), (nk_final_waves<T, true, 2, FinalTile<T, NL, 2, 2>::THREADS>()))
+    k2_final_g(NkPassF p, NkGroupFuse fa, NkGroupWork wa, int count, int64_t per, const C2<T>* __restrict__ tw, int xmap) {
+  extern __shared__ __align__(16) unsigned char smem[];
+  int64_t member, local;
+  nk_group_decode((int64_t)blockIdx.x, count, member, local);
+  if (local >= per) return;
+  DeviceExec<T, SchedF<T, NL>::E> ex;
+  double acc = 0.0;
+  float wmax = 0.0f;
+  const int64_t blk = xmap ? nk_xcd_contig(local, per) : local;
+  nk_final_body<T, NL, FinalTile<T, NL, 2, 2>::TILE, true, 2, 1>(ex, p, fa.f[member], blk, (T*)smem, tw, (const C2<T>*)wa.work[member], &acc,
+                                                                &wmax);
+  nk_group_flush(fa.f[member], acc, wmax, local);
+}
+
+template <typename T, int NL>
+int nk_group_launch_final(NkPassF pf, const NkGroupFuse& fa, const NkGroupWork& wa, int count, const C2<T>* tw, hipStream_t st) {
+  using CT = FinalTile<T, NL, 2, 2>;
+  static_assert(CT::TILE >= 2, "the couple (b0, M - b0) must live in one workgroup");
+  if (pf.a_cnt > 0 || pf.g.batch != 1) return nk_set_error(NK_ERR_UNSUPPORTED, "grouped final pass: one unstaged grid per member");
+  pf.tiles_per_a = pf.A > 1 ? (pf.M / 2 + 1 + CT::TILE / 2 - 1) / (CT::TILE / 2) : (pf.M + CT::TILE - 1) / CT::TILE;
+  pf.blk0 = 0;
+  const int64_t per = (int64_t)(pf.A / 2 + 1) * pf.tiles_per_a;
+  const int64_t grid = nk_group_grid(per, count);
+  if (grid > 0x7fffffffLL) return nk_set_error(NK_ERR_UNSUPPORTED, "too many lines for one launch");
+  for (int m = 0; m < count; ++m)
+    if (fa.f[m].value_slots > 0 && per * ((CT::THREADS + 63) / 64) > fa.f[m].value_slots)
+      return nk_set_error(NK_ERR_RUNTIME, "final pass: more wavefronts than reduction slots (nk_value_slot_count)");
+  return nk_launch<k2_final_g<T, NL>>("k2_final_g", dim3((unsigned)grid), dim3(CT::THREADS), CT::LDS_BYTES, st, pf, fa, wa, count, per, tw,
+                                      nk_knobs().xmap & 4);
+}
+
+#define NK_CASE(NN)                                                                                                                       \
+  template int nk_group_launch_contig3<float, NN, 5>(const NkPass3&, const NkGroupFuse&, const NkGroupWork&, int, const C2<float>*,        \
+                                                     const C2<float>*, hipStream_t);                                                      \
+  template int nk_group_launch_contig3<float, NN, 8>(const NkPass3&, const NkGroupFuse&, const NkGroupWork&, int, const C2<float>*,        \
+                                                     const C2<float>*, hipStream_t);                                                      \
+  template int nk_group_launch_contig3<double, NN, 5>(const NkPass3&, const NkGroupFuse&, const NkGroupWork&, int, const C2<double>*,      \
+                                                      const C2<double>*, hipStream_t);                                                    \
+  template int nk_group_launch_contig3<double, NN, 8>(const NkPass3&, const NkGroupFuse&, const NkGroupWork&, int, const C2<double>*,      \
+                                                      const C2<double>*, hipStream_t);                                                    \
+  template int nk_group_launch_final<float, NN>(NkPassF, const NkGroupFuse&, const NkGroupWork&, int, const C2<float>*, hipStream_t);      \
+  template int nk_group_launch_final<double, NN>(NkPassF, const NkGroupFuse&, const NkGroupWork&, int, const C2<double>*, hipStream_t);
+NK_FAST_SIZES(NK_CASE)
+#undef NK_CASE
diff --git a/nifty_amd/csrc/nk_plan.h b/nifty_amd/csrc/nk_plan.h
--- a/nifty_amd/csrc/nk_plan.h
+++ b/nifty_amd/csrc/nk_plan.h
@@ -62,6 +62,7 @@
   int mid_wg_per_cu = 0;
   int pair_hand = 0;
   int pair_pad_lds = 0;
+  int group = 1;
   int tile_divides = 0;
 };
 static inline NkKnobs nk_read_knobs() {
@@ -78,6 +79,7 @@
   k.mid_wg_per_cu = nk_env_int("NK_MID_WG_PER_CU", k.mid_wg_per_cu);
   k.pair_hand = nk_env_int("NK_PAIR_HAND", k.pair_hand);
   k.pair_pad_lds = nk_env_int("NK_PAIR_PAD_LDS", k.pair_pad_lds);
+  k.group = nk_env_int("NK_GROUP", k.group);
   k.tile_divides = nk_env_int("NK_TILE_DIVIDES", k.tile_divides);
   return k;
 }
diff --git a/nifty_amd/engine.py b/nifty_amd/engine.py
--- a/nifty_amd/engine.py
+++ b/nifty_amd/engine.py
@@ -914,6 +914,68 @@
                     "nk_octant_scatter_k2")
             self._finish_metric(lp, d, out, is_first, ident, dest)
 
+    def group_ready(self):
+        return bool(self.pair_ready() and self.fused_direction and os.environ.get("NK_GROUP", "1") != "0"
+                    and os.environ.get("NK_DA_GATHER", "0") != "1")
+
+    def _group_buffers(self, count):
+        own = dict(damp=self.damp, dafield=self.dafield, w8=self.w8, w8max=self.w8max, workspace=self.plan.workspace)
+        sets = [own, self._pair_buffers()] if count > 1 else [own]
+        more = self.__dict__.setdefault("_group_more", [])
+        while len(sets) + len(more) < count:
+            more.append(dict(damp=torch.empty_like(self.damp), dafield=torch.empty_like(self.dafield),
+                             w8=torch.empty_like(self.w8), w8max=torch.zeros_like(self.w8max),
+                             workspace=torch.empty_like(self.plan.workspace)))
+        return (sets + more)[:count]
+
+    def release_group_buffers(self):
+        self.__dict__.pop("_group_more", None)
+
+    def lh_metric_group(self, lp, jobs):
+        lib = L.load()
+        bufs = self._group_buffers(len(jobs))
+        fuses, outs, adds = [], [], []
+        points = [job.get("lp", lp) for job in jobs]
+        for job, buf, lp in zip(jobs, bufs, points):
+            d = job["d"]
+            avec, afac = (d, job.get("identity", 0.0)) if job.get("addend") is None else job["addend"]
+            out = LatentVec(torch.empty_like(d.xi), None)
+            L.check(lib.nk_amp_jvp(self.nb, self.geo.data_ptr(), self.hyp.data_ptr(), lp.x.small.data_ptr(), lp.state.data_ptr(),
+                                   d.small.data_ptr(), buf["damp"].data_ptr(), B._stream()), "nk_amp_jvp")
+            self._amp_field(buf["damp"], out=buf["dafield"])
+            f = self._fuse()
+            f.pro, f.in_, f.in2 = L.PRO_AMP_JVP, d.xi.data_ptr(), lp.x.xi.data_ptr()
+            f.pidx, f.amp, f.damp = self.pidx.data_ptr(), lp.amp.data_ptr(), buf["damp"].data_ptr()
+            f.afield, f.dafield = B.ptr(lp.afield), buf["dafield"].data_ptr()
+            if job.get("cg_direction") is not None:
+                f.cg_r, f.cg_scal = job["cg_direction"][0].xi.data_ptr(), job["cg_direction"][1].scal.data_ptr()
+            f.mul, f.mul_scalar = B.ptr(lp.mid), lp.mid_scalar
+            f.epi, f.out, f.scale = L.EPI_VJP, out.xi.data_ptr(), self.h_dvol
+            f.xi = lp.x.xi.data_ptr()
+            f.addend, f.addend_scale, f.accumulate = B.ptr(avec.xi if afac else None), afac, 0
+            if job.get("dot_out") is not None:
+                if not afac:
+                    raise ValueError("dot_out needs an addend and the register-resident transform pipeline")
+                f.value = job["dot_out"].data_ptr()
+            f.abar, f.w8 = self.abar.data_ptr(), buf["w8"].data_ptr()
+            if self.scatter_fixed_point:
+                f.w8max = buf["w8max"].data_ptr()
+            fuses.append(f)
+            outs.append(out)
+            adds.append((avec, afac))
+        B.hartley_sandwich_group(self.plan, fuses, self.h_dvol, [buf["workspace"] for buf in bufs])
+        shp = (ctypes.c_int64 * len(self.shape))(*self.shape)
+        for job, buf, out, (avec, afac), lp in zip(jobs, bufs, outs, adds, points):
+            self._count("transforms", 2)
+            L.check(lib.nk_octant_scatter_k2(len(self.shape), shp, buf["w8"].data_ptr(), self.pidx.data_ptr(), self.bin_k2.data_ptr(),
+                                             self.nb, self.scatter_scratch.data_ptr(), self.abar.data_ptr(),
+                                             buf["w8max"].data_ptr() if self.scatter_fixed_point else 0, B._stream()),
+                    "nk_octant_scatter_k2")
+            if job.get("cg_direction") is not None:
+                job["cg_direction"][1].roll()
+            self._finish_metric(lp, avec, out, True, afac, _Dest(out.xi, accumulate=False))
+        return outs
+
     def _finish_metric(self, lp, d, out, first, identity, dest=None):
         self._amp_vjp(lp)
         if dest is not None:
@@ -1592,7 +1654,19 @@
     local_pairs = len({i // 2 if plan.mirror else i for i in range(plan.lo, plan.hi)})
     lanes = _sampling_lanes(model, local_pairs)
     in_batch = local_pairs >= 2 and batched.ready(model)
-    if lanes is None and not in_batch:
+    grouped = (lanes is None and not in_batch and local_pairs >= 2 and geo_minimizer is None and model.group_ready()
+               and model.N > int(os.environ.get("NK_LANE_MAX_POINTS", str(1 << 25))))
+    if grouped:
+        if want_ahead:
+            ahead = _HostDrawAhead(model, drawn_seeds)
+        try:
+            drawn = plan.run_together(
+                lambda seed: _draw_sources(model, linearisation(), seed, device_rng, ahead.take(seed) if ahead else None),
+                lambda jobs: _solve_grouped(model, linearisation(), jobs, controller_factory), finish)
+        finally:
+            if ahead is not None:
+                ahead.close()
+    elif lanes is None and not in_batch:
         if want_ahead:
             ahead = _HostDrawAhead(model, drawn_seeds)
         try:
@@ -1689,10 +1763,80 @@
     return model.lanes(min(want, pairs))
 
 
-def _draw_sources(model, lp, seed, device_rng):
+def _draw_sources(model, lp, seed, device_rng, ahead=None):
     if device_rng is not None:
         device_rng.manual_seed(int(seed.generate_state(1, np.uint64)[0] >> np.uint64(1)))
-    return model.draw_prior(device_rng), model.draw_lh_noise(lp, device_rng)
+    return model.draw_prior(device_rng, ahead=ahead), model.draw_lh_noise(lp, device_rng)
+
+
+class _Ticket:
+
+    __slots__ = ("job", "result")
+
+    def __init__(self, job):
+        self.job, self.result = job, None
+
+
+class _GroupedMetric:
+
+    fused_dot = fused_direction = True
+
+    def __init__(self, model, lp, size):
+        self._model, self._lp, self._size, self._queue = model, lp, size, []
+
+    def __call__(self, v, dot_out=None, cg_direction=None):
+        return self._model.metric(self._lp, v, dot_out=dot_out, cg_direction=cg_direction)
+
+    def submit(self, v, dot_out=None, cg_direction=None):
+        ticket = _Ticket(dict(d=v, identity=1.0, dot_out=dot_out, cg_direction=cg_direction))
+        self._queue.append(ticket)
+        return ticket
+
+    def flush(self):
+        queue, self._queue = self._queue, []
+        for with_direction in (False, True):
+            part = [t for t in queue if (t.job["cg_direction"] is not None) == with_direction]
+            for k in range(0, len(part), self._size):
+                chunk = part[k:k + self._size]
+                for ticket, out in zip(chunk, self._model.lh_metric_group(self._lp, [t.job for t in chunk])):
+                    ticket.result = out
+
+
+def _solve_grouped(model, lp, jobs, controller_factory):
+    import copy
+
+    size = max(1, min(L.MAX_GROUP, int(os.environ.get("NK_GROUP_SOLVES", str(L.MAX_GROUP)))))
+    pairs = []
+    for w0 in range(0, len(jobs), size):
+        wave = jobs[w0:w0 + size]
+        bs = [s + nj for s, nj in wave]
+        g0s = model.lh_metric_group(lp, [dict(d=s, addend=(nj, -1.0)) for s, nj in wave])
+        starts = [s for s, _ in wave]
+        jobs[w0:w0 + size] = [None] * len(wave)
+        del wave
+        op = _GroupedMetric(model, lp, size)
+        runs, controllers = [], []
+        for s, b, g0 in zip(starts, bs, g0s):
+            energy = QuadraticEnergy(s, op, b, _grad=g0)
+            energy.consumable = True
+            controller = controller_factory()
+            if any(controller is other for other in controllers):
+                controller = copy.deepcopy(controller)
+            controllers.append(controller)
+            runs.append(ConjugateGradient(None)._inplace_steps(energy, controller))
+        results, active = [None] * len(runs), list(range(len(runs)))
+        while active:
+            for k in list(active):
+                try:
+                    next(runs[k])
+                except StopIteration as done:
+                    results[k] = done.value
+                    active.remove(k)
+            op.flush()
+        pairs += [(b, energy.position) for b, (energy, _) in zip(bs, results)]
+        del runs, results, starts, g0s, op
+    model.release_group_buffers()
+    return pairs
 
 
 def _solve_on_lanes(model, lanes, lp, jobs, controller_factory):
diff --git a/nifty_amd/minimization.py b/nifty_amd/minimization.py
--- a/nifty_amd/minimization.py
+++ b/nifty_amd/minimization.py
@@ -488,6 +488,14 @@
         fused_dot = bool(getattr(A, "fused_dot", False)) and hasattr(ws, "curv_slot")
         fused_dir = bool(getattr(A, "fused_direction", False)) and hasattr(ws, "direction_small")
 
+        def apply(v, **kw):
+            submit = getattr(A, "submit", None)
+            if submit is None:
+                return A(v, **kw)
+            ticket = submit(v, **kw)
+            yield ticket
+            return ticket.result
+
         def device_iteration(with_direction):
             extra = {}
             if with_direction and fused_dir:
@@ -496,10 +504,10 @@
             elif with_direction:
                 ws.direction(d, r)
             if fused_dot:
-                q = A(d, dot_out=ws.curv_slot(), **extra)
+                q = yield from apply(d, dot_out=ws.curv_slot(), **extra)
                 ws.curv_small(d, q)
             else:
-                q = A(d, **extra)
+                q = yield from apply(d, **extra)
                 ws.curv(d, q)
             if track_energy:
                 ws.update_dr(x, r, d, q)
@@ -511,13 +519,13 @@
         iteration = 0
         while True:
             iteration += 1
-            device_iteration(iteration > 1 and not direction_done)
+            yield from device_iteration(iteration > 1 and not direction_done)
             direction_done = False
             counters.add("cg_iterations")
             since_reset += 1
             refreshed = False
             if since_reset >= self._nreset and not _forced_stop(controller):
-                Ax = A(x)
+                Ax = yield from apply(x)
                 r = Ax - b if b is not None else Ax
                 ws.refresh(x, r, b)
                 since_reset = 0
```

Result: faster. 0.2209 (median of 6 runs) (+3.7%).
